# MyrtleSoftware/myrtlespeech

Hardware: AMD Instinct MI355X
Metric: audio-sec/s (RTF), DS2 5xBiLSTM-1024 encoder forward + CTC greedy, 80-feature 10 s clips @ batch 32/GPU (higher is better)
Workload: dtype f16x3 (f32 split in fp16 hi+lo, 3 fp16 MFMA passes, f32 acc: LSTM, projections, conv1/2, FC1; FC2/CTC/decode f32)

## Files before the change

include/ms_hotpath.h:

```cpp
#ifndef MS_HOTPATH_H
#define MS_HOTPATH_H

#include <stddef.h>
#include <stdint.h>

#ifdef __cplusplus
extern "C" {
#endif

#define MS_ABI_VERSION 4

enum {
  MS_OK = 0,
  MS_ERR_INVALID = 1,
  MS_ERR_HIP = 2,
  MS_ERR_WORKSPACE = 3,
  MS_ERR_TIMEOUT = 4,
  MS_ERR_UNSUPPORTED = 5
};

enum { MS_CELL_LSTM = 0, MS_CELL_GRU = 1, MS_CELL_RNN_TANH = 2, MS_CELL_HARD_LSTM = 3 };

enum { MS_ACT_NONE = 0, MS_ACT_CLAMP = 1  };

int ms_abi_version(void);
const char* ms_last_error(void);


int ms_mask_time_(float* x, const int32_t* lens, int N, int inner, int T, void* stream);

size_t ms_maskconv_packed_bytes(int Cout, int Cin_g, int KF, int KT, int groups);

int ms_maskconv_pack(const float* w, void* packed, int Cout, int Cin_g, int KF, int KT, int groups, void* stream);

int ms_maskconv_forward(const float* x, const int32_t* lens, const void* packed_w, const float* bias, float* y,
                        int N, int Cin, int Fin, int Tin, int Cout, int Fout, int Tout, int KF, int KT, int SF,
                        int ST, int DF, int DT, int pad_f_l, int pad_t_l, int groups, int act, float act_lo,
                        float act_hi, void* stream);

size_t ms_maskconv_cl_packed_bytes(int Cout, int Cin, int KF, int KT);
int ms_maskconv_cl_pack(const float* w, void* packed, int Cout, int Cin, int KF, int KT, void* stream);
size_t ms_maskconv_cl_workspace_bytes(int N, int Cin, int Fin, int Tin);
int ms_maskconv_cl_forward(const float* x, const int32_t* lens, const void* packed_w, const float* bias, float* y,
                           int N, int Cin, int Fin, int Tin, int Cout, int Fout, int Tout, int KF, int KT, int SF,
                           int ST, int DF, int DT, int pad_f_l, int pad_t_l, int act, float act_lo, float act_hi,
                           void* workspace, size_t workspace_bytes, void* stream);

size_t ms_maskconv_fwin_packed_bytes(int Cout, int KF, int KT);
int ms_maskconv_fwin_pack(const float* w, void* packed, int Cout, int KF, int KT, void* stream);
size_t ms_maskconv_fwin_workspace_bytes(int N, int Tin, int KF, int SF, int Fout);
int ms_maskconv_fwin_forward(const float* x, const int32_t* lens, const void* packed_w, const float* bias, float* y, int N,
                             int Fin, int Tin, int Cout, int Fout, int Tout, int KF, int KT, int SF, int ST, int DT,
                             int pad_f_l, int pad_t_l, int act, float act_lo, float act_hi, void* workspace,
                             size_t workspace_bytes, void* stream);

size_t ms_maskconv1d_gemm_packed_bytes(int Cout, int Cin, int KT);
int ms_maskconv1d_gemm_pack(const float* w, void* packed, int Cout, int Cin, int KT, void* stream);
size_t ms_maskconv1d_gemm_workspace_bytes(int N, int Cin, int Tout, int Cout, int KT);
int ms_maskconv1d_gemm_forward(const float* x, const int32_t* lens, const void* packed, const float* bias, float* y, int N,
                               int Cin, int Tin, int Cout, int Tout, int KT, int ST, int DT, int pad_l, int act,
                               float act_lo, float act_hi, void* workspace, size_t workspace_bytes, void* stream);

int ms_nct_to_tnc(const float* x, float* y, int N, int CF, int T, void* stream);

int ms_clamp(const float* x, float* y, size_t n, float lo, float hi, void* stream);


int ms_linear_forward(const float* x, const float* w, const float* bias, float* y, int M, int K, int N, int act,
                      float act_lo, float act_hi, void* stream);

#define MS_LINEAR_FEW_ROWS 1
size_t ms_linear_splitk_workspace_bytes(int M, int K, int N, int flags);
int ms_linear_splitk_forward(const float* x, const float* w, const float* bias, float* y, int M, int K, int N, int act,
                             float act_lo, float act_hi, int flags, void* workspace, size_t workspace_bytes, void* stream);

size_t ms_linear_split_workspace_bytes(int M, int K, int N);
int ms_linear_split_forward(const float* x, const float* w, const float* bias, float* y, int M, int K, int N, int act,
                            float act_lo, float act_hi, void* workspace, size_t workspace_bytes, void* stream);

size_t ms_linear_split_packed_bytes(int K, int N);
int ms_linear_split_pack(const float* w, void* packed, int K, int N, void* stream);
int ms_linear_split_forward_packed(const float* x, const void* packed_w, const float* bias, float* y, int M, int K, int N, int act,
                                   float act_lo, float act_hi, void* workspace, size_t workspace_bytes, void* stream);


int ms_lookahead_forward(const float* x, const float* w, float* y, int N, int F, int T, int ctx, long xs_n,
                         long xs_f, long xs_t, long ys_n, long ys_f, long ys_t, int act, float act_lo,
                         float act_hi, void* stream);

int ms_lookahead_window_forward(const float* x, const float* w, float* y, int N, int F, int T_in, int T_out, int ctx,
                                long xs_n, long xs_f, long xs_t, long ys_n, long ys_f, long ys_t, int act, float act_lo,
                                float act_hi, void* stream);


int ms_rnn_padded_hidden(int cell, int H, int ndir);
size_t ms_rnn_packed_bytes(int cell, int In, int H, int ndir);
int ms_rnn_pack(int cell, int In, int H, int ndir, const float* const* w_ih_host, const float* const* w_hh_host,
                const float* const* b_ih_host, const float* const* b_hh_host, void* packed, void* stream);

size_t ms_rnn_workspace_bytes(int cell, int T, int N, int In, int H, int ndir);

int ms_rnn_layer_forward(int cell, const void* packed, const float* x, const int32_t* lens, int max_len,
                         const float* h0, const float* c0, float* out, float* hn, float* cn, int T, int N, int In,
                         int H, int ndir, void* workspace, size_t workspace_bytes, void* stream);

enum { MS_RNN_X_PLANES_IN_WS = 1, MS_RNN_OUT_PLANES_TO_WS = 2, MS_RNN_PACKED_ROWS = 4, MS_RNN_HX_PREINIT = 4096,
       MS_RNN_RECURRENCE_ONLY = 8192, MS_RNN_TIMING_SKIP_PROJECTION = 8192 ,
       MS_RNN_PROJECTION_ONLY = 16384 };
int ms_rnn_layer_chains_planes(int cell, int H, int ndir);
int ms_rnn_hx_preinit(int cell, int T, int N, int In, int H, int ndir, int max_len, int nregions, void* workspace,
                      size_t workspace_bytes, void* stream);
int ms_rnn_layer_packs_rows(int cell, int T, int N, int In, int H, int ndir);
int ms_rnn_layer_forward_ex(int cell, const void* packed, const float* x, const int32_t* lens, int max_len,
                            const float* h0, const float* c0, float* out, float* hn, float* cn, int T, int N, int In,
                            int H, int ndir, int flags, void* workspace, size_t workspace_bytes, void* stream);

int ms_rnn_layer_is_wide(int cell, int H, int ndir, int N);
int ms_rnn_stack_overlap_ok(int cell, int T, int N, int In, int H, int ndir, int nl);
int ms_rnn_stack_forward(int cell, const void* const* packed_host, const float* x, const int32_t* lens, int max_len,
                         const float* h0, const float* c0, float* out, float* hn, float* cn, int T, int N, int In, int H, int ndir,
                         int nl, int segments, void* workspace, size_t workspace_bytes, void* stream);

int ms_rnn_status(const void* workspace, void* stream);

size_t ms_rnn_debug_offset(int cell, int T, int N, int In, int H, int ndir);

int ms_gemm_set_variant(int variant);

enum {
  MS_PROF_PROJECTION = 0, MS_PROF_RECURRENCE = 1, MS_PROF_GEMM_K_LARGE = 2, MS_PROF_GEMM_K_SMALL = 3, MS_PROF_CONV = 4,
  MS_PROF_LAYOUT = 5, MS_PROF_LINEAR = 6, MS_PROF_GREEDY = 7, MS_PROF_OTHER = 8
};
#define MS_PROF_KINDS 9
int ms_prof_enable(int on);
int ms_prof_read(float* out_ms_host, int* out_n_host);

int ms_clock_probe(unsigned long long* out_dev, int samples, int spacing_us, void* stream);

int ms_barrier_chain_probe(unsigned long long* out_dev, int steps, int threads, void* stream);


size_t ms_ctc_loss_workspace_bytes(int T, int N, int V, int S_max);

int ms_ctc_status(const void* workspace, void* stream);

#define MS_CTC_LOG_PROBS_IN 2
int ms_ctc_loss_forward(const float* logits, const int32_t* in_lens, const int32_t* targets,
                        const int32_t* tgt_offsets, const int32_t* tgt_lens, float* nll, float* reduced, int T,
                        int N, int V, int S_max, int blank, int reduction, int zero_infinity, void* workspace,
                        size_t workspace_bytes, void* stream);

int ms_log_softmax_axis(const float* x, float* y, int outer, int axis, int inner, void* stream);
int ms_log_softmax_axis_backward(const float* y, const float* g, float* gx, int outer, int axis, int inner, void* stream);

size_t ms_ctc_loss_backward_workspace_bytes(int T, int N, int V, int S_max);
int ms_ctc_loss_backward(const float* logits, const int32_t* in_lens, const int32_t* targets, const int32_t* tgt_offsets,
                         const int32_t* tgt_lens, const float* grad_nll, float* grad_logits, int T, int N, int V,
                         int S_max, int blank, int zero_infinity, void* workspace, size_t workspace_bytes, void* stream);


int ms_ctc_greedy_decode(const float* x, const int32_t* lens, int32_t* out_idx, int32_t* out_len, int T, int N,
                         int V, int blank, void* stream);

size_t ms_ctc_greedy_stream_state_bytes(int N);
int ms_ctc_greedy_stream_begin(void* state, int N, void* stream);
int ms_ctc_greedy_stream_step(const float* x, int rows, int n, int V, int blank, const int32_t* total_lens,
                              const int32_t* chunk_lens, int32_t* labels, int32_t* label_frames, int cap, int32_t* fresh,
                              void* state, int N, void* stream);


#define MS_CTC_ALIGN_BP_LDS_BYTES 98304
size_t ms_ctc_align_workspace_bytes(int T, int N, int V, int S_max);
int ms_ctc_align(const float* x, const int32_t* in_lens, const int32_t* targets, const int32_t* tgt_offsets,
                 const int32_t* tgt_lens, float* score, int32_t* frame_state, int32_t* token_start, int32_t* token_end,
                 float* token_logp, int T, int N, int V, int L_max, int blank, int flags, void* workspace,
                 size_t workspace_bytes, void* stream);


size_t ms_ctc_beam_workspace_bytes(int T, int N, int V, int beam_width);

int ms_ctc_beam_decode(const float* probs, const int32_t* lens, int32_t* out_idx, int32_t* out_len, int T, int N,
                       int V, int blank, int beam_width, float prune_threshold, int separator, const float* word_factor,
                       int t_begin, int t_end, const float* lm_factor, int finish, int32_t* beam_len,
                       int32_t* beam_idx, int32_t* beam_plen, void* workspace, size_t workspace_bytes,
                       void* stream);

int ms_ctc_beam_decode_rows(const float* probs, const int32_t* lens, int32_t* out_idx, int32_t* out_len, int T, int N,
                            int V, int blank, int beam_width, float prune_threshold, int separator,
                            const float* word_factor, int t_begin, int t_end, int row0, int rows_held,
                            const float* lm_factor, int finish, int32_t* beam_len, int32_t* beam_idx, int32_t* beam_plen,
                            void* workspace, size_t workspace_bytes, void* stream);


#define MS_NGRAM_MAX_ORDER 5

int ms_ngram_lm_table_check(const void* blob_host, size_t bytes);

int ms_ngram_lm_score(const void* table, const void* header_host, size_t table_bytes, const int32_t* prefixes,
                      const int32_t* prefix_lens, float* out, int P, int L, int separator, void* stream);

size_t ms_ctc_beam_lm_workspace_bytes(int T, int N, int V, int beam_width, int order);
int ms_ctc_beam_decode_lm(const float* probs, const int32_t* lens, int32_t* out_idx, int32_t* out_len, int T, int N,
                          int V, int blank, int beam_width, float prune_threshold, int separator,
                          const float* word_factor, int t_begin, int t_end, int row0, int rows_held, const void* lm_table,
                          const void* lm_header_host, size_t lm_table_bytes, int finish, int32_t* beam_len,
                          int32_t* beam_idx, int32_t* beam_plen, void* workspace, size_t workspace_bytes, void* stream);

int ms_ctc_beam_decode_ex(const float* probs, const int32_t* lens, int32_t* out_idx, int32_t* out_len, int T, int N,
                          int V, int blank, int beam_width, float prune_threshold, int separator,
                          const float* word_factor, int t_begin, int t_end, int row0, int rows_held,
                          const float* lm_factor, int finish, int32_t* beam_len, int32_t* beam_idx, int32_t* beam_plen,
                          void* workspace, size_t workspace_bytes, void* stream, const void* lm_table,
                          const void* lm_header_host, size_t lm_table_bytes, int range_safe, float* beam_score,
                          int32_t* scale_log2);


size_t ms_mfcc_workspace_bytes(int N, int T, int n_fft, int n_mels, int n_mfcc);
int ms_mfcc_forward(const float* wave, const int32_t* wave_lens, const float* window, const float* dft,
                    const float* mel_fb, const float* dct, float* out, int N, int max_samples, int T, int n_fft,
                    int hop, int n_mels, int n_mfcc, float top_db, void* workspace, size_t workspace_bytes,
                    void* stream);

int ms_mfcc_legacy_forward(const float* wave, const int32_t* wave_lens, const double* twiddle, const double* fbank,
                           const double* dct, const double* lifter, float* out, int N, int max_samples, int T,
                           int frame_len, int frame_step, int nfft, int nfilt, int numcep, double preemph,
                           void* stream);

size_t ms_standardize_workspace_bytes(int N);
int ms_standardize_forward(const float* x, const int32_t* lens, float* y, int N, int inner, int T, void* workspace,
                           size_t workspace_bytes, void* stream);

int ms_context_frames_forward(const float* x, const int32_t* lens, float* y, int N, int F, int T, int n_context,
                              void* stream);

int ms_spec_augment_(float* x, const int32_t* f_bands, const int32_t* t_bands, int N, int C, int F, int T, int n_f,
                     int n_t, void* stream);


int ms_embedding_forward(const float* table, const int32_t* idx, float* out, int R, int D, int V1, void* stream);

int ms_rnnt_joint_forward(const float* enc_p, const int32_t* enc_row, const float* pred_p, const float* w_out,
                          const float* b_out, float* logp, int R, int J, int V1, void* stream);

int ms_rnnt_topk(const float* scores, int32_t* out_idx, float* out_val, int B, int C, int k, void* stream);

size_t ms_rnnt_decode_workspace_bytes(int T, int N, int V, int D, int H, int L, int J, int beam_width, int max_symbols,
                                      int greedy);
int ms_rnnt_decode(const float* enc_p, const int32_t* lens, const float* embedding, const float* const* w_ih,
                   const float* const* w_hh, const float* const* b_ih, const float* const* b_hh, const float* w_pred,
                   const float* w_out, const float* b_out, int32_t* out_idx, int32_t* out_len, float* out_score, int T,
                   int N, int V, int D, int H, int L, int J, int beam_width, int max_symbols, int greedy, void* workspace,
                   size_t workspace_bytes, void* stream);

size_t ms_rnnt_loss_lattice_bytes(int N, int T, int U1);
size_t ms_rnnt_loss_workspace_bytes(int N, int T, int U1, int V1);
int ms_rnnt_loss_forward(const float* logits, const int32_t* in_lens, const int32_t* targets, const int32_t* tgt_lens,
                         float* nll, float* lattice, int N, int T, int U1, int V1, int blank, void* workspace,
                         size_t workspace_bytes, void* stream);
int ms_rnnt_loss_backward(const float* logits, const int32_t* in_lens, const int32_t* targets, const int32_t* tgt_lens,
                          const float* nll, const float* lattice, const float* grad_nll, float* grad, int N, int T, int U1,
                          int V1, int blank, void* stream);

size_t ms_rnnt_score_lattice_bytes(int N, int T, int U1);
size_t ms_rnnt_score_workspace_bytes(int N, int T, int U1, int J, int V1);
int ms_rnnt_score(const float* enc_p, const float* pred_p, const float* w_out, const float* b_out, const int32_t* in_lens,
                  const int32_t* targets, const int32_t* tgt_lens, float* nll, float* lattice, int N, int T, int U1, int J,
                  int V1, int blank, void* workspace, size_t workspace_bytes, void* stream);

#ifdef __cplusplus
}
#endif
#endif
```

myrtlespeech_amd/_lib.py:

```python
import ctypes
import os
import re
from ctypes import POINTER, c_char_p, c_double, c_float, c_int, c_int32, c_long, c_size_t, c_void_p

import torch

_HERE = os.path.dirname(os.path.abspath(__file__))
LIB_PATH = os.environ.get("MS_HOTPATH_LIB") or os.path.join(_HERE, "libms_hotpath.so")
HEADER_PATH = os.path.join(os.path.dirname(_HERE), "include", "ms_hotpath.h")

MS_OK = 0
ABI_VERSION = 4
ERR_NAMES = {1: "MS_ERR_INVALID", 2: "MS_ERR_HIP", 3: "MS_ERR_WORKSPACE", 4: "MS_ERR_TIMEOUT", 5: "MS_ERR_UNSUPPORTED"}

CELL_LSTM, CELL_GRU, CELL_RNN_TANH, CELL_HARD_LSTM = 0, 1, 2, 3
ACT_NONE, ACT_CLAMP = 0, 1
LINEAR_FEW_ROWS = 1
PROF_KINDS = 9

_P = c_void_p
_PP = POINTER(c_void_p)

SIGNATURES = {
    "ms_abi_version": (c_int, []),
    "ms_last_error": (c_char_p, []),
    "ms_mask_time_": (c_int, [_P, _P, c_int, c_int, c_int, _P]),
    "ms_maskconv_packed_bytes": (c_size_t, [c_int, c_int, c_int, c_int, c_int]),
    "ms_maskconv_pack": (c_int, [_P, _P, c_int, c_int, c_int, c_int, c_int, _P]),
    "ms_maskconv_forward": (c_int, [_P, _P, _P, _P, _P] + [c_int] * 17 + [c_float, c_float, _P]),
    "ms_maskconv_cl_packed_bytes": (c_size_t, [c_int, c_int, c_int, c_int]),
    "ms_maskconv_cl_pack": (c_int, [_P, _P, c_int, c_int, c_int, c_int, _P]),
    "ms_maskconv_cl_workspace_bytes": (c_size_t, [c_int, c_int, c_int, c_int]),
    "ms_maskconv_cl_forward": (c_int, [_P, _P, _P, _P, _P] + [c_int] * 16 + [c_float, c_float, _P, c_size_t, _P]),
    "ms_maskconv_fwin_packed_bytes": (c_size_t, [c_int, c_int, c_int]),
    "ms_maskconv_fwin_pack": (c_int, [_P, _P, c_int, c_int, c_int, _P]),
    "ms_maskconv_fwin_workspace_bytes": (c_size_t, [c_int, c_int, c_int, c_int, c_int]),
    "ms_maskconv_fwin_forward": (c_int, [_P, _P, _P, _P, _P] + [c_int] * 14 + [c_float, c_float, _P, c_size_t, _P]),
    "ms_maskconv1d_gemm_packed_bytes": (c_size_t, [c_int, c_int, c_int]),
    "ms_maskconv1d_gemm_pack": (c_int, [_P, _P, c_int, c_int, c_int, _P]),
    "ms_maskconv1d_gemm_workspace_bytes": (c_size_t, [c_int] * 5),
    "ms_maskconv1d_gemm_forward": (c_int, [_P, _P, _P, _P, _P] + [c_int] * 10 + [c_float, c_float, _P, c_size_t, _P]),
    "ms_nct_to_tnc": (c_int, [_P, _P, c_int, c_int, c_int, _P]),
    "ms_clamp": (c_int, [_P, _P, c_size_t, c_float, c_float, _P]),
    "ms_linear_forward": (c_int, [_P, _P, _P, _P, c_int, c_int, c_int, c_int, c_float, c_float, _P]),
    "ms_linear_splitk_workspace_bytes": (c_size_t, [c_int, c_int, c_int, c_int]),
    "ms_linear_splitk_forward": (c_int, [_P, _P, _P, _P, c_int, c_int, c_int, c_int, c_float, c_float, c_int, _P, c_size_t, _P]),
    "ms_linear_split_workspace_bytes": (c_size_t, [c_int, c_int, c_int]),
    "ms_linear_split_forward": (c_int, [_P, _P, _P, _P, c_int, c_int, c_int, c_int, c_float, c_float, _P, c_size_t, _P]),
    "ms_linear_split_packed_bytes": (c_size_t, [c_int, c_int]),
    "ms_linear_split_pack": (c_int, [_P, _P, c_int, c_int, _P]),
    "ms_linear_split_forward_packed": (c_int, [_P, _P, _P, _P, c_int, c_int, c_int, c_int, c_float, c_float, _P, c_size_t, _P]),
    "ms_lookahead_forward": (c_int, [_P, _P, _P, c_int, c_int, c_int, c_int] + [c_long] * 6 + [c_int, c_float, c_float, _P]),
    "ms_lookahead_window_forward": (c_int, [_P, _P, _P, c_int, c_int, c_int, c_int, c_int] + [c_long] * 6 + [c_int, c_float, c_float, _P]),
    "ms_rnn_packed_bytes": (c_size_t, [c_int, c_int, c_int, c_int]),
    "ms_ctc_status": (c_int, [_P, _P]),
    "ms_rnn_padded_hidden": (c_int, [c_int, c_int, c_int]),
    "ms_rnn_hx_preinit": (c_int, [c_int] * 8 + [_P, c_size_t, _P]),
    "ms_rnn_pack": (c_int, [c_int, c_int, c_int, c_int, _PP, _PP, _PP, _PP, _P, _P]),
    "ms_rnn_workspace_bytes": (c_size_t, [c_int] * 6),
    "ms_rnn_layer_forward": (c_int, [c_int, _P, _P, _P, c_int, _P, _P, _P, _P, _P] + [c_int] * 5 + [_P, c_size_t, _P]),
    "ms_rnn_layer_forward_ex": (c_int, [c_int, _P, _P, _P, c_int, _P, _P, _P, _P, _P] + [c_int] * 6 + [_P, c_size_t, _P]),
    "ms_rnn_layer_chains_planes": (c_int, [c_int, c_int, c_int]),
    "ms_rnn_layer_is_wide": (c_int, [c_int] * 4),
    "ms_rnn_stack_overlap_ok": (c_int, [c_int] * 7),
    "ms_rnn_stack_forward": (c_int, [c_int, _P, _P, _P, c_int, _P, _P, _P, _P, _P] + [c_int] * 7 + [_P, c_size_t, _P]),
    "ms_rnn_status": (c_int, [_P, _P]),
    "ms_rnn_debug_offset": (c_size_t, [c_int] * 6),
    "ms_rnn_layer_packs_rows": (c_int, [c_int] * 6),
    "ms_gemm_set_variant": (c_int, [c_int]),
    "ms_prof_enable": (c_int, [c_int]),
    "ms_prof_read": (c_int, [POINTER(c_float), POINTER(c_int)]),
    "ms_clock_probe": (c_int, [_P, c_int, c_int, _P]),
    "ms_barrier_chain_probe": (c_int, [_P, c_int, c_int, _P]),
    "ms_ctc_loss_workspace_bytes": (c_size_t, [c_int] * 4),
    "ms_ctc_loss_forward": (c_int, [_P] * 7 + [c_int] * 7 + [_P, c_size_t, _P]),
    "ms_log_softmax_axis": (c_int, [_P, _P, c_int, c_int, c_int, _P]),
    "ms_log_softmax_axis_backward": (c_int, [_P, _P, _P, c_int, c_int, c_int, _P]),
    "ms_ctc_loss_backward_workspace_bytes": (c_size_t, [c_int] * 4),
    "ms_ctc_loss_backward": (c_int, [_P] * 7 + [c_int] * 6 + [_P, c_size_t, _P]),
    "ms_ctc_greedy_decode": (c_int, [_P, _P, _P, _P, c_int, c_int, c_int, c_int, _P]),
    "ms_ctc_align_workspace_bytes": (c_size_t, [c_int] * 4),
    "ms_ctc_align": (c_int, [_P] * 10 + [c_int] * 6 + [_P, c_size_t, _P]),
    "ms_ctc_greedy_stream_state_bytes": (c_size_t, [c_int]),
    "ms_ctc_greedy_stream_begin": (c_int, [_P, c_int, _P]),
    "ms_ctc_greedy_stream_step": (c_int, [_P, c_int, c_int, c_int, c_int, _P, _P, _P, _P, c_int, _P, _P, c_int, _P]),
    "ms_embedding_forward": (c_int, [_P, _P, _P, c_int, c_int, c_int, _P]),
    "ms_rnnt_joint_forward": (c_int, [_P, _P, _P, _P, _P, _P, c_int, c_int, c_int, _P]),
    "ms_rnnt_topk": (c_int, [_P, _P, _P, c_int, c_int, c_int, _P]),
    "ms_ctc_beam_workspace_bytes": (c_size_t, [c_int] * 4),
    "ms_ctc_beam_decode": (c_int, [_P, _P, _P, _P, c_int, c_int, c_int, c_int, c_int, c_float, c_int, _P, c_int, c_int,
                                   _P, c_int, _P, _P, _P, _P, c_size_t, _P]),
    "ms_ctc_beam_decode_rows": (c_int, [_P, _P, _P, _P, c_int, c_int, c_int, c_int, c_int, c_float, c_int, _P, c_int, c_int,
                                        c_int, c_int, _P, c_int, _P, _P, _P, _P, c_size_t, _P]),
    "ms_ngram_lm_table_check": (c_int, [_P, c_size_t]),
    "ms_ngram_lm_score": (c_int, [_P, _P, c_size_t, _P, _P, _P, c_int, c_int, c_int, _P]),
    "ms_ctc_beam_lm_workspace_bytes": (c_size_t, [c_int] * 5),
    "ms_ctc_beam_decode_lm": (c_int, [_P, _P, _P, _P, c_int, c_int, c_int, c_int, c_int, c_float, c_int, _P, c_int, c_int,
                                      c_int, c_int, _P, _P, c_size_t, c_int, _P, _P, _P, _P, c_size_t, _P]),
    "ms_ctc_beam_decode_ex": (c_int, [_P, _P, _P, _P, c_int, c_int, c_int, c_int, c_int, c_float, c_int, _P, c_int, c_int,
                                      c_int, c_int, _P, c_int, _P, _P, _P, _P, c_size_t, _P, _P, _P, c_size_t, c_int, _P, _P]),
    "ms_rnnt_decode_workspace_bytes": (c_size_t, [c_int] * 10),
    "ms_rnnt_decode": (c_int, [_P, _P, _P, _PP, _PP, _PP, _PP, _P, _P, _P, _P, _P, _P] + [c_int] * 10 + [_P, c_size_t, _P]),
    "ms_rnnt_loss_lattice_bytes": (c_size_t, [c_int] * 3),
    "ms_rnnt_loss_workspace_bytes": (c_size_t, [c_int] * 4),
    "ms_rnnt_loss_forward": (c_int, [_P] * 6 + [c_int] * 5 + [_P, c_size_t, _P]),
    "ms_rnnt_loss_backward": (c_int, [_P] * 8 + [c_int] * 5 + [_P]),
    "ms_rnnt_score_lattice_bytes": (c_size_t, [c_int] * 3),
    "ms_rnnt_score_workspace_bytes": (c_size_t, [c_int] * 5),
    "ms_rnnt_score": (c_int, [_P] * 9 + [c_int] * 6 + [_P, c_size_t, _P]),
    "ms_mfcc_workspace_bytes": (c_size_t, [c_int] * 5),
    "ms_mfcc_forward": (c_int, [_P] * 7 + [c_int] * 7 + [c_float, _P, c_size_t, _P]),
    "ms_mfcc_legacy_forward": (c_int, [_P] * 7 + [c_int] * 8 + [c_double, _P]),
    "ms_standardize_workspace_bytes": (c_size_t, [c_int]),
    "ms_standardize_forward": (c_int, [_P, _P, _P, c_int, c_int, c_int, _P, c_size_t, _P]),
    "ms_context_frames_forward": (c_int, [_P, _P, _P, c_int, c_int, c_int, c_int, _P]),
    "ms_spec_augment_": (c_int, [_P, _P, _P] + [c_int] * 6 + [_P]),
}

_lib = None


def header_symbols():
    with open(HEADER_PATH) as f:
        text = re.sub(r"/\*.*?\*/", "", f.read(), flags=re.S)
    return sorted(set(re.findall(r"\b(ms_[a-z0-9_]+)\s*\(", text)))


def load():
    global _lib
    if _lib is None:
        if not os.path.exists(LIB_PATH):
            raise RuntimeError(
                f"{LIB_PATH} not found: build it with `python -c 'import __graft_entry__ as g; g.build()'` "
                "(or `make -C myrtlespeech_amd/csrc`). There is no CPU fallback."
            )
        lib = ctypes.CDLL(LIB_PATH)
        for name, (res, args) in SIGNATURES.items():
            fn = getattr(lib, name)
            fn.restype = res
            fn.argtypes = args
        got = lib.ms_abi_version()
        if got != ABI_VERSION:
            raise RuntimeError(f"{LIB_PATH} reports MS_ABI_VERSION {got}, this binding needs {ABI_VERSION}: rebuild the "
                               "library (`make -C myrtlespeech_amd/csrc`)")
        _lib = lib
    return _lib


def require_gpu():
    if not torch.cuda.is_available():
        raise RuntimeError("myrtlespeech_amd: a HIP device (MI355X) is required; there is no CPU fallback")


def stream_ptr():
    return c_void_p(torch.cuda.current_stream().cuda_stream)


def ptr(t, strided=False):
    if t is None:
        return c_void_p(0)
    if not isinstance(t, torch.Tensor):
        raise TypeError(f"_lib.ptr: expected a torch.Tensor or None, got {type(t).__name__}")
    if not t.is_cuda:
        raise ValueError(f"_lib.ptr: a {t.device.type} tensor (shape {tuple(t.shape)}) cannot be a device-pointer argument; "
                         "move it to the GPU first (host buffers go through _lib.host_ptr)")
    if not strided and not t.is_contiguous():
        raise ValueError(f"_lib.ptr: tensor of shape {tuple(t.shape)} and strides {tuple(t.stride())} is not contiguous; the "
                         "kernels read dense storage (call .contiguous())")
    return c_void_p(t.data_ptr())


def host_ptr(t):
    if t is None:
        return c_void_p(0)
    if not isinstance(t, torch.Tensor) or t.is_cuda or not t.is_contiguous():
        raise ValueError("_lib.host_ptr: expected a contiguous CPU tensor")
    return c_void_p(t.data_ptr())


def check(rc, what):
    if rc != MS_OK:
        msg = load().ms_last_error().decode()
        raise RuntimeError(f"{what} failed with {ERR_NAMES.get(rc, rc)}: {msg}")


def f32c(t):
    if t.dtype != torch.float32:
        t = t.float()
    if not t.is_cuda:
        t = t.cuda()
    return t.contiguous()


_ASYNC_LENS = os.environ.get("MS_ASYNC_LENS") != "0"


_const_lens = {}


def _const_tensor(shape, dtype, value, make: bool):
    key = (tuple(shape), dtype, int(value))
    rec = _const_lens.get(key)
    if rec is not None:
        t, version = rec
        if version_of(t) == version:
            return t
        _const_lens[("stale", len(_const_lens)) + key] = rec
        del _const_lens[key]
    if not make or len(_const_lens) >= 4096:
        return None
    t = torch.full(tuple(shape), int(value), dtype=dtype, device="cuda")
    _const_lens[key] = (t, version_of(t))
    return t


def _all_equal_value(h: torch.Tensor):
    if h.numel() == 0 or h.numel() > 4096 or h.dtype not in (torch.int32, torch.int64):
        return None
    flat = h.reshape(-1)
    v = int(flat[0])
    return v if bool((flat == v).all()) else None


def upload(host: torch.Tensor, dtype=None) -> torch.Tensor:
    h = host.detach()
    if dtype is not None and h.dtype != dtype:
        h = h.to(dtype)
    h = h.contiguous()
    if torch.cuda.is_available() and torch.cuda.is_current_stream_capturing():
        flat = h.reshape(-1)
        if flat.numel() and bool((flat == flat[0]).all()):
            c = _const_tensor(h.shape, h.dtype, flat[0].item(), make=False) if h.dtype in (torch.int32, torch.int64) else None
            return c if c is not None else torch.full(h.shape, flat[0].item(), dtype=h.dtype, device="cuda")
        raise RuntimeError("host values that differ cannot be uploaded inside a HIP graph capture")
    if torch.cuda.is_available():
        v = _all_equal_value(h)
        if v is not None:
            _const_tensor(h.shape, h.dtype, v, make=True)
    if not _ASYNC_LENS:
        return h.cuda()
    try:
        h = h.pin_memory()
    except RuntimeError:
        return h.cuda()
    return h.to("cuda", non_blocking=True)


def attach_host(dev: torch.Tensor, host: torch.Tensor) -> torch.Tensor:
    dev._ms_host = (host.detach().clone(), version_of(dev), dev.data_ptr())
    return dev


def version_of(t: torch.Tensor) -> int:
    return -1 if t.is_inference() else t._version


def host_lens(lens: torch.Tensor) -> torch.Tensor:
    if not lens.is_cuda:
        return lens.detach().to(torch.int64)
    h = cached_host(lens) if _ASYNC_LENS else None
    if h is not None:
        return h.to(torch.int64)
    return lens.detach().to("cpu", torch.int64)


def cached_host(lens: torch.Tensor):
    rec = getattr(lens, "_ms_host", None)
    if rec is None:
        return None
    h, version, address = rec
    if h.shape == lens.shape and version == version_of(lens) and address == lens.data_ptr():
        return h
    lens._ms_host = None
    return None


def lens_to_device(lens: torch.Tensor) -> torch.Tensor:
    if lens.is_cuda:
        return lens
    return attach_host(upload(lens), lens.detach())


def lens_i32(lens):
    if lens.is_cuda:
        if lens.dtype == torch.int32 and lens.is_contiguous():
            return lens
        h = cached_host(lens) if _ASYNC_LENS else None
        if h is not None:
            v = _all_equal_value(h)
            if v is not None:
                c = _const_tensor(lens.shape, torch.int32, v, make=not torch.cuda.is_current_stream_capturing())
                if c is not None and torch.cuda.is_current_stream_capturing():
                    return c
        return lens.to(torch.int32).contiguous()
    return upload(lens, torch.int32)


def split_precision():
    return os.environ.get("MS_PRECISION") != "f32"


issue_point = None


def at_issue_point():
    hook = issue_point
    if hook is not None:
        hook()


class Workspace:

    def __init__(self):
        self.buf = None

    def get(self, nbytes, zero: bool = True):
        if self.buf is None or self.buf.numel() < nbytes:
            make = torch.zeros if zero else torch.empty
            self.buf = make(max(int(nbytes), 256), dtype=torch.uint8, device="cuda")
        return self.buf
```

myrtlespeech_amd/csrc/conv_cl.hip:

```cpp
#include <algorithm>
#include <type_traits>

#include "common.h"

namespace {

typedef unsigned u32x4 __attribute__((ext_vector_type(4)));
typedef unsigned u32x2 __attribute__((ext_vector_type(2)));
typedef __bf16 bf16x8 __attribute__((ext_vector_type(8)));
typedef _Float16 f16x8 __attribute__((ext_vector_type(8)));

constexpr int CL_F = 2;

struct ClP {
  int N, Cin, Fin, Tin, Cout, Fout, Tout, KF, KT, SF, ST, DF, DT, pad_f, pad_t;
  int KG;
  int PW;
  int co_tiles;
  int act;
  float lo, hi;
  int FP;
};

__device__ __forceinline__ unsigned bf16b(float x) { return (unsigned)__builtin_bit_cast(unsigned short, (__bf16)x); }
__device__ __forceinline__ unsigned f16b(float x) { return (unsigned)__builtin_bit_cast(unsigned short, (_Float16)x); }
__device__ __forceinline__ void split_by_prec(float x, int prec, unsigned& hi, unsigned& lo) {
  if (prec == ms::PREC_F16) { hi = f16b(x); lo = 0u; }
  else if (prec == ms::PREC_F16X3) ms::plane_split<true>(x, hi, lo);
  else ms::plane_split<false>(x, hi, lo);
}

__global__ void conv_cl_pack_kernel(const float* __restrict__ w, unsigned short* __restrict__ packed, int Cout, int Cin,
                                    int KF, int KT, int cout_pad, int prec, const float* __restrict__ scale_word) {
  const int KG = Cin / 8;
  const float wscale = scale_word[0];
  const size_t plane = (size_t)KF * KT * KG * cout_pad * 8;
  for (size_t i = (size_t)blockIdx.x * blockDim.x + threadIdx.x; i < plane; i += (size_t)gridDim.x * blockDim.x) {
    const int e = i & 7;
    const int co = (i >> 3) % cout_pad;
    const int kg = (i / ((size_t)8 * cout_pad)) % KG;
    const int kt = (i / ((size_t)8 * cout_pad * KG)) % KT;
    const int kf = i / ((size_t)8 * cout_pad * KG * KT);
    float x = 0.f;
    if (co < Cout) x = w[(((size_t)co * Cin + kg * 8 + e) * KF + kf) * KT + kt] * wscale;
    unsigned h, l;
    split_by_prec(x, prec, h, l);
    packed[i] = (unsigned short)h;
    packed[plane + i] = (unsigned short)l;
  }
}

template <int P, bool WIN = false, int WF = 1>
__global__ __launch_bounds__(256, 2) void maskconv_cl_kernel(const unsigned short* __restrict__ xh,
                                                             const unsigned short* __restrict__ xl,
                                                             const int32_t* __restrict__ lens,
                                                             const unsigned short* __restrict__ wp,
                                                             const float* __restrict__ bias, float* __restrict__ y, ClP p,
                                                             const float* __restrict__ scale_word) {
  constexpr bool F16 = ms::prec_one_plane(P), HM = P == ms::PREC_F16X3;
  constexpr int WT = 4 / WF;
  constexpr int TT = 32 * WT;
  constexpr int RF = CL_F * WF;
  extern __shared__ __attribute__((aligned(16))) char lds[];
  const int row_bytes = p.KG * p.PW * 16;
  char* Ph = lds;
  char* Pl = lds + RF * row_bytes;
  char* Wh = lds + 2 * RF * row_bytes;
  const int wtap = p.KG * 32 * 16;
  char* Wl = Wh + ((p.KT + 1) / 2) * wtap;

  const int tid = threadIdx.x, lane = tid & 63, wave = tid >> 6;
  const int l31 = lane & 31, half = lane >> 5;
  const int wt = wave % WT, wf = wave / WT;
  const int t0 = blockIdx.x * TT;
  const int fo0 = blockIdx.y * RF;
  const int n = blockIdx.z / p.co_tiles, tile = blockIdx.z % p.co_tiles;
  const int len = lens ? min(lens[n], p.Tin) : p.Tin;
  const int cout_pad = p.co_tiles * 32;
  const size_t wplane = (size_t)p.KF * p.KT * p.KG * cout_pad * 8;

  ms::f32x16 acc[CL_F];
#pragma unroll
  for (int f = 0; f < CL_F; ++f)
#pragma unroll
    for (int r = 0; r < 16; ++r) acc[f][r] = 0.f;

  const int tin0 = t0 * p.ST - p.pad_t;
  const int ngran = p.KG * p.PW;
  const unsigned plane_bytes = WIN ? (unsigned)((size_t)p.N * p.Tin * p.FP * 2) : 0u;
  const __amdgpu_buffer_rsrc_t xh_rsrc = __builtin_amdgcn_make_buffer_rsrc(const_cast<unsigned short*>(xh), 0, plane_bytes, 0x00020000);
  const __amdgpu_buffer_rsrc_t xl_rsrc = __builtin_amdgcn_make_buffer_rsrc(const_cast<unsigned short*>(xl), 0, plane_bytes, 0x00020000);

  for (int kf = 0; kf < p.KF; ++kf) {
    for (int f = 0; f < RF; ++f) {
      const int fin = (fo0 + f) * p.SF - p.pad_f + kf * p.DF;
      const bool frow = (fo0 + f) < p.Fout && (WIN || (fin >= 0 && fin < p.Fin));
      const size_t rbase = ((size_t)n * p.Fin + (frow && !WIN ? fin : 0)) * p.Tin;
      for (int i = tid; i < ngran; i += 256) {
        const int q = i / p.KG, kg = i - q * p.KG;
        const int tin = tin0 + q;
        u32x4 vh = {0u, 0u, 0u, 0u}, vl = {0u, 0u, 0u, 0u};
        if (frow && tin >= 0 && tin < len) {
          if (WIN) {
            const int boff = (int)((((size_t)n * p.Tin + tin) * p.FP + (size_t)(fo0 + f) * p.SF + kg * 8) * 2);
            vh = __builtin_amdgcn_raw_buffer_load_b128(xh_rsrc, boff, 0, 0);
            if (!F16) vl = __builtin_amdgcn_raw_buffer_load_b128(xl_rsrc, boff, 0, 0);
          } else {
            const size_t off = (rbase + tin) * p.Cin + kg * 8;
            vh = *reinterpret_cast<const u32x4*>(xh + off);
            if (!F16) vl = *reinterpret_cast<const u32x4*>(xl + off);
          }
        }
        *reinterpret_cast<u32x4*>(Ph + f * row_bytes + (kg * p.PW + q) * 16) = vh;
        if (!F16) *reinterpret_cast<u32x4*>(Pl + f * row_bytes + (kg * p.PW + q) * 16) = vl;
      }
    }
    const int taps_per_stage = (p.KT + 1) / 2;
    for (int kt0 = 0; kt0 < p.KT; kt0 += taps_per_stage) {
      const int ntap = min(taps_per_stage, p.KT - kt0);
      if (kt0 > 0) __syncthreads();
      {
        const int ng = ntap * p.KG * 32;
        for (int i = tid; i < ng; i += 256) {
          const int co = i & 31, rest = i >> 5;
          const size_t src = ((((size_t)kf * p.KT + kt0) * p.KG + rest) * cout_pad + tile * 32 + co) * 8;
          *reinterpret_cast<u32x4*>(Wh + i * 16) = *reinterpret_cast<const u32x4*>(wp + src);
          if (!F16) *reinterpret_cast<u32x4*>(Wl + i * 16) = *reinterpret_cast<const u32x4*>(wp + wplane + src);
        }
      }
      __syncthreads();
      for (int ktl = 0; ktl < ntap; ++ktl) {
        const int tq = (wt * 32 + l31) * p.ST + (kt0 + ktl) * p.DT;
        for (int s = 0; s < p.KG / 2; ++s) {
          const int kg = 2 * s + half;
          const int woff = ((ktl * p.KG + kg) * 32 + l31) * 16;
          const u32x4 ah = *reinterpret_cast<const u32x4*>(Wh + woff);
          u32x4 al = ah;
          if (!F16) al = *reinterpret_cast<const u32x4*>(Wl + woff);
#pragma unroll
          for (int f = 0; f < CL_F; ++f) {
            const int poff = (wf * CL_F + f) * row_bytes + (kg * p.PW + tq) * 16;
            const u32x4 bh = *reinterpret_cast<const u32x4*>(Ph + poff);
            if (F16) {
              acc[f] = __builtin_amdgcn_mfma_f32_32x32x16_f16(__builtin_bit_cast(f16x8, ah), __builtin_bit_cast(f16x8, bh), acc[f], 0, 0, 0);
            } else {
              const u32x4 bl = *reinterpret_cast<const u32x4*>(Pl + poff);
              acc[f] = ms::mfma_32x32x16<HM>(ah, bh, acc[f]);
              acc[f] = ms::mfma_32x32x16<HM>(al, bh, acc[f]);
              acc[f] = ms::mfma_32x32x16<HM>(ah, bl, acc[f]);
            }
          }
        }
      }
    }
    __syncthreads();
  }

  const int t = t0 + wt * 32 + l31;
  const float winv = scale_word[1];
  if (t < p.Tout) {
#pragma unroll
    for (int f = 0; f < CL_F; ++f) {
      const int fo = fo0 + wf * CL_F + f;
      if (fo >= p.Fout) continue;
#pragma unroll
      for (int r = 0; r < 16; ++r) {
        const int co = tile * 32 + ms::mfma32_row(r, lane);
        if (co < p.Cout) {
          float v = acc[f][r] * winv + (bias ? bias[co] : 0.f);
          if (p.act == MS_ACT_CLAMP) v = fminf(fmaxf(v, p.lo), p.hi);
          y[(((size_t)n * p.Cout + co) * p.Fout + fo) * p.Tout + t] = v;
        }
      }
    }
  }
}


constexpr int SH_RB = 12;
constexpr int SH_KT = 11;

template <int P>
__global__ __launch_bounds__(256, 1) void maskconv_cl_short_kernel(const unsigned short* __restrict__ xh,
                                                                   const unsigned short* __restrict__ xl,
                                                                   const int32_t* __restrict__ lens,
                                                                   const unsigned short* __restrict__ wp,
                                                                   const float* __restrict__ bias, float* __restrict__ y, ClP p,
                                                                   int RB, int RIN, const float* __restrict__ scale_word) {
  constexpr bool F16 = ms::prec_one_plane(P), HM = P == ms::PREC_F16X3;
  const float winv = scale_word[1];
  extern __shared__ __attribute__((aligned(16))) char lds[];
  const int tid = threadIdx.x, lane = tid & 63, wave = __builtin_amdgcn_readfirstlane(tid >> 6);
  const int c16 = lane & 15, q = lane >> 4;
  const int fo0 = blockIdx.x * RB, cb = blockIdx.y, n = blockIdx.z;
  const int PW = p.PW;
  const int row_bytes = PW * 64;
  char* Ph = lds;
  char* Pl = lds + (size_t)RIN * row_bytes;
  const int len = lens ? min(lens[n], p.Tin) : p.Tin;
  const int fin_lo = fo0 * p.SF - p.pad_f;

  for (int i = tid; i < RIN * PW * 4; i += 256) {
    const int kg = i & 3, rq = i >> 2;
    const int r = rq / PW, fq = rq - r * PW;
    const int fin = fin_lo + r, tin = fq - p.pad_t;
    u32x4 vh = {0u, 0u, 0u, 0u}, vl = {0u, 0u, 0u, 0u};
    if (fin >= 0 && fin < p.Fin && tin >= 0 && tin < len) {
      const size_t off = (((size_t)n * p.Fin + fin) * p.Tin + tin) * 32 + kg * 8;
      vh = *reinterpret_cast<const u32x4*>(xh + off);
      if (!F16) vl = *reinterpret_cast<const u32x4*>(xl + off);
    }
    *reinterpret_cast<u32x4*>(Ph + r * row_bytes + fq * 64 + kg * 16) = vh;
    if (!F16) *reinterpret_cast<u32x4*>(Pl + r * row_bytes + fq * 64 + kg * 16) = vl;
  }
  __syncthreads();

  ms::f32x4 acc[SH_RB];
#pragma unroll
  for (int i = 0; i < SH_RB; ++i) acc[i] = ms::f32x4{0.f, 0.f, 0.f, 0.f};
  const int cout_pad = p.co_tiles * 32;
  const size_t wplane = (size_t)p.KF * p.KT * 4 * cout_pad * 8;
  const unsigned short* wa = wp + (size_t)q * cout_pad * 8 + (cb * 16 + c16) * 8;
  const size_t tap_stride = (size_t)4 * cout_pad * 8;
  u32x4 fh[2][SH_KT], fl[2][SH_KT];
  auto load_row = [&](auto set, int kf) {
#pragma unroll
    for (int kt = 0; kt < SH_KT; ++kt)
      if (kt < p.KT) {
        const unsigned short* src = wa + (size_t)(kf * p.KT + kt) * tap_stride;
        fh[set][kt] = *reinterpret_cast<const u32x4*>(src);
        if (!F16) fl[set][kt] = *reinterpret_cast<const u32x4*>(src + wplane);
      }
  };
  auto compute_row = [&](auto set, int kf) {
#pragma unroll
    for (int i = 0; i < SH_RB; ++i) {
      const int fo = fo0 + i;
      const int fin = fo * p.SF - p.pad_f + kf * p.DF;
      if (i < RB && fo < p.Fout && fin >= 0 && fin < p.Fin) {
        const int rbase = (fin - fin_lo) * row_bytes + c16 * 64 + q * 16;
#pragma unroll
        for (int kt = 0; kt < SH_KT; ++kt)
          if (kt < p.KT) {
            const u32x4 bh = *reinterpret_cast<const u32x4*>(Ph + rbase + kt * 64);
            if (F16) {
              acc[i] = __builtin_amdgcn_mfma_f32_16x16x32_f16(__builtin_bit_cast(f16x8, fh[set][kt]), __builtin_bit_cast(f16x8, bh), acc[i], 0, 0, 0);
            } else {
              const u32x4 bl = *reinterpret_cast<const u32x4*>(Pl + rbase + kt * 64);
              acc[i] = ms::mfma_16x16x32<HM>(fh[set][kt], bh, acc[i]);
              acc[i] = ms::mfma_16x16x32<HM>(fl[set][kt], bh, acc[i]);
              acc[i] = ms::mfma_16x16x32<HM>(fh[set][kt], bl, acc[i]);
            }
          }
      }
    }
  };
  constexpr std::integral_constant<int, 0> S0{};
  constexpr std::integral_constant<int, 1> S1{};
  if (wave < p.KF) load_row(S0, wave);
  for (int kf = wave; kf < p.KF; kf += 8) {
    if (kf + 4 < p.KF) load_row(S1, kf + 4);
    compute_row(S0, kf);
    if (kf + 8 < p.KF) load_row(S0, kf + 8);
    if (kf + 4 < p.KF) compute_row(S1, kf + 4);
  }

  __syncthreads();
  ms::f32x4* part = reinterpret_cast<ms::f32x4*>(lds);
#pragma unroll
  for (int i = 0; i < SH_RB; ++i)
    if (i < RB) part[(wave * SH_RB + i) * 64 + lane] = acc[i];
  __syncthreads();
#pragma unroll
  for (int j = 0; j < SH_RB / 4; ++j) {
    const int i = wave + 4 * j, fo = fo0 + i;
    if (i >= RB || fo >= p.Fout) continue;
    ms::f32x4 v = part[(0 * SH_RB + i) * 64 + lane];
#pragma unroll
    for (int w = 1; w < 4; ++w) v += part[(w * SH_RB + i) * 64 + lane];
    if (c16 < p.Tout) {
#pragma unroll
      for (int r = 0; r < 4; ++r) {
        const int co = cb * 16 + 4 * q + r;
        if (co < p.Cout) {
          float o = v[r] * winv + (bias ? bias[co] : 0.f);
          if (p.act == MS_ACT_CLAMP) o = fminf(fmaxf(o, p.lo), p.hi);
          y[(((size_t)n * p.Cout + co) * p.Fout + fo) * p.Tout + c16] = o;
        }
      }
    }
  }
}

int conv_cl_short_plan(const ClP& p, bool f16, int* RB, int* RIN, size_t* lds) {
  static const bool off = getenv("MS_CONV_SHORT") && getenv("MS_CONV_SHORT")[0] == '0';
  if (off || p.Cin != 32 || p.Tout > 16 || p.ST != 1 || p.DT != 1 || p.FP != 0 || p.N > 65535 || p.KT > SH_KT) return 0;
  const int cbs = ms::cdiv(p.Cout, 16);
  int nblk = std::max(1, std::min(ms::cdiv(p.Fout, 4), ms::cdiv(ms::num_cus(), p.N * cbs)));
  while (ms::cdiv(p.Fout, nblk) > SH_RB) ++nblk;
  for (; nblk <= p.Fout; ++nblk) {
    const int rb = ms::cdiv(p.Fout, nblk);
    const int rin = (rb - 1) * p.SF + (p.KF - 1) * p.DF + 1;
    const size_t bytes = std::max((size_t)(f16 ? 1 : 2) * rin * (p.Tout + p.KT - 1) * 64, (size_t)4 * SH_RB * 64 * 16);
    if (bytes <= 156 * 1024) { *RB = rb; *RIN = rin; *lds = bytes; return 1; }
  }
  return 0;
}

__global__ void nchw_to_cl_split_kernel(const float* __restrict__ x, unsigned short* __restrict__ hi,
                                        unsigned short* __restrict__ lo, int C, int F, int T, int prec) {
  __shared__ float tile[32][33];
  const int n = blockIdx.z / F, f = blockIdx.z % F;
  const int t0 = blockIdx.x * 32, c0 = blockIdx.y * 32;
  const int tx = threadIdx.x, ty = threadIdx.y;
  for (int i = ty; i < 32; i += 8) {
    const int c = c0 + i, t = t0 + tx;
    tile[i][tx] = (c < C && t < T) ? x[(((size_t)n * C + c) * F + f) * T + t] : 0.f;
  }
  __syncthreads();
  for (int i = ty; i < 32; i += 8) {
    const int t = t0 + i, c = c0 + tx;
    if (t < T && c < C) {
      const float v = tile[tx][i];
      const size_t o = (((size_t)n * F + f) * T + t) * C + c;
      unsigned h, l;
      split_by_prec(v, prec, h, l);
      hi[o] = (unsigned short)h;
      if (prec != ms::PREC_F16) lo[o] = (unsigned short)l;
    }
  }
}

__global__ void ft_to_tf_split_kernel(const float* __restrict__ x, unsigned short* __restrict__ hi,
                                      unsigned short* __restrict__ lo, int Fin, int T, int FP, int pad, int prec) {
  __shared__ float tile[32][33];
  const int n = blockIdx.z;
  const int t0 = blockIdx.x * 32, j0 = blockIdx.y * 32;
  const int tx = threadIdx.x, ty = threadIdx.y;
  for (int i = ty; i < 32; i += 8) {
    const int fidx = j0 + i - pad, t = t0 + tx;
    tile[i][tx] = (fidx >= 0 && fidx < Fin && t < T) ? x[((size_t)n * Fin + fidx) * T + t] : 0.f;
  }
  __syncthreads();
  for (int i = ty; i < 32; i += 8) {
    const int t = t0 + i, j = j0 + tx;
    if (t < T && j < FP) {
      const float v = tile[tx][i];
      const size_t o = ((size_t)n * T + t) * FP + j;
      unsigned h, l;
      split_by_prec(v, prec, h, l);
      hi[o] = (unsigned short)h;
      if (prec != ms::PREC_F16) lo[o] = (unsigned short)l;
    }
  }
}

__global__ void conv_fwin_pack_kernel(const float* __restrict__ w, unsigned short* __restrict__ packed, int Cout, int KF,
                                      int KT, int KG, int cout_pad, int prec, const float* __restrict__ scale_word) {
  const size_t plane = (size_t)KT * KG * cout_pad * 8;
  const float wscale = scale_word[0];
  for (size_t i = (size_t)blockIdx.x * blockDim.x + threadIdx.x; i < plane; i += (size_t)gridDim.x * blockDim.x) {
    const int e = i & 7;
    const int co = (i >> 3) % cout_pad;
    const int kg = (i / ((size_t)8 * cout_pad)) % KG;
    const int kt = i / ((size_t)8 * cout_pad * KG);
    const int kf = kg * 8 + e;
    float x = 0.f;
    if (co < Cout && kf < KF) x = w[((size_t)co * KF + kf) * KT + kt] * wscale;
    unsigned h, l;
    split_by_prec(x, prec, h, l);
    packed[i] = (unsigned short)h;
    packed[plane + i] = (unsigned short)l;
  }
}

int conv_cl_plan(ClP& p, size_t* lds) {
  const size_t wbytes = (size_t)2 * ((p.KT + 1) / 2) * p.KG * 32 * 16;
  if ((long)p.N * p.co_tiles > 65535) return 0;
  for (int wf : {p.Tout <= 48 ? 4 : 1, 1}) {
    const int tt = 128 / wf, rf = CL_F * wf;
    p.PW = (tt - 1) * p.ST + (p.KT - 1) * p.DT + 1;
    *lds = (size_t)2 * rf * p.KG * p.PW * 16 + wbytes;
    if (*lds <= 160 * 1024 && ms::cdiv(p.Fout, rf) <= 65535) return wf;
  }
  return 0;
}

template <bool WIN>
int conv_cl_launch(const ClP& p, int wf, size_t lds, const unsigned short* xh, const unsigned short* xl, const int32_t* lens,
                   const void* packed_w, const float* bias, float* y, hipStream_t stream, const float* scale_word) {
  static ms::DeviceOnce attr_once;
  if (attr_once.need()) {
#define MS_CL_ATTR(PP)                                                                                                                     \
    MS_HIP(hipFuncSetAttribute((const void*)maskconv_cl_kernel<PP, WIN, 1>, hipFuncAttributeMaxDynamicSharedMemorySize, 160 * 1024));   \
    MS_HIP(hipFuncSetAttribute((const void*)maskconv_cl_kernel<PP, WIN, 4>, hipFuncAttributeMaxDynamicSharedMemorySize, 160 * 1024));
    MS_CL_ATTR(ms::PREC_BF16X3) MS_CL_ATTR(ms::PREC_F16) MS_CL_ATTR(ms::PREC_F16X3)
#undef MS_CL_ATTR
    attr_once.done();
  }
  const int prec = ms::split_mode();
  const int tt = 128 / wf, rf = CL_F * wf;
  dim3 grid(ms::cdiv(p.Tout, tt), ms::cdiv(p.Fout, rf), p.N * p.co_tiles);
  const unsigned short* wq = (const unsigned short*)packed_w;
#define MS_CL_LAUNCH(WF_)                                                                                                             \
  if (prec == ms::PREC_F16) hipLaunchKernelGGL((maskconv_cl_kernel<ms::PREC_F16, WIN, WF_>), grid, dim3(256), lds, stream, xh, xl, lens, wq, bias, y, p, scale_word); \
  else if (prec == ms::PREC_F16X3) hipLaunchKernelGGL((maskconv_cl_kernel<ms::PREC_F16X3, WIN, WF_>), grid, dim3(256), lds, stream, xh, xl, lens, wq, bias, y, p, scale_word); \
  else hipLaunchKernelGGL((maskconv_cl_kernel<ms::PREC_BF16X3, WIN, WF_>), grid, dim3(256), lds, stream, xh, xl, lens, wq, bias, y, p, scale_word);
  if (wf == 4) { MS_CL_LAUNCH(4) } else { MS_CL_LAUNCH(1) }
#undef MS_CL_LAUNCH
  MS_LAUNCH_CHECK();
  return MS_OK;
}

inline int fwin_kfp(int KF) { return ms::cdiv(KF, 16) * 16; }
inline int fwin_fp(int KF, int SF, int Fout) { return ms::cdiv((Fout - 1) * SF + fwin_kfp(KF), 32) * 32; }

}

static size_t fwin_plane_bytes(int Cout, int KF, int KT) {
  return ms::align_up((size_t)2 * KT * (fwin_kfp(KF) / 8) * (ms::cdiv(Cout, 32) * 32) * 8 * sizeof(unsigned short), 256);
}
extern "C" size_t ms_maskconv_fwin_packed_bytes(int Cout, int KF, int KT) {
  if (Cout <= 0 || KF <= 0 || KT <= 0) return 0;
  return fwin_plane_bytes(Cout, KF, KT) + 256;
}

extern "C" int ms_maskconv_fwin_pack(const float* w, void* packed, int Cout, int KF, int KT, void* stream) {
  MS_REQUIRE(w && packed, "null pointer");
  MS_REQUIRE(Cout > 0 && KF > 0 && KT > 0, "bad shape");
  const int cout_pad = ms::cdiv(Cout, 32) * 32, KG = fwin_kfp(KF) / 8;
  const size_t plane = (size_t)KT * KG * cout_pad * 8;
  const int blocks = (int)std::min<size_t>((plane + 255) / 256, 2048);
  float* scale_word = (float*)((char*)packed + fwin_plane_bytes(Cout, KF, KT));
  const int rc = ms::weight_scale_launch(w, (size_t)Cout * KF * KT, scale_word, ms::split_mode(), (hipStream_t)stream);
  if (rc != MS_OK) return rc;
  hipLaunchKernelGGL(conv_fwin_pack_kernel, dim3(blocks), dim3(256), 0, (hipStream_t)stream, w, (unsigned short*)packed, Cout,
                     KF, KT, KG, cout_pad, ms::split_mode(), scale_word);
  MS_LAUNCH_CHECK();
  return MS_OK;
}

extern "C" size_t ms_maskconv_fwin_workspace_bytes(int N, int Tin, int KF, int SF, int Fout) {
  if (N <= 0 || Tin <= 0 || KF <= 0 || SF <= 0 || Fout <= 0) return 0;
  return ms::align_up((size_t)N * Tin * fwin_fp(KF, SF, Fout) * 4, 256);
}

extern "C" int ms_maskconv_fwin_forward(const float* x, const int32_t* lens, const void* packed_w, const float* bias, float* y,
                                        int N, int Fin, int Tin, int Cout, int Fout, int Tout, int KF, int KT, int SF, int ST,
                                        int DT, int pad_f_l, int pad_t_l, int act, float act_lo, float act_hi, void* workspace,
                                        size_t workspace_bytes, void* stream_) {
  ms::ProfScope prof_span(MS_PROF_CONV, (hipStream_t)stream_);
  MS_REQUIRE(x && packed_w && y && workspace, "null pointer");
  MS_REQUIRE(N > 0 && Fin > 0 && Tin > 0 && Cout > 0 && Fout > 0 && Tout > 0, "bad shape");
  MS_REQUIRE(KF > 0 && KT > 0 && SF > 0 && ST > 0 && DT > 0 && pad_f_l >= 0 && pad_t_l >= 0, "bad kernel");
  MS_REQUIRE(SF % 2 == 0, "feature stride must be even (4-byte aligned window loads)");
  MS_REQUIRE(act == MS_ACT_NONE || act == MS_ACT_CLAMP, "bad act");
  if (workspace_bytes < ms_maskconv_fwin_workspace_bytes(N, Tin, KF, SF, Fout)) {
    ms::set_error("ms_maskconv_fwin_forward: workspace too small");
    return MS_ERR_WORKSPACE;
  }
  hipStream_t stream = (hipStream_t)stream_;
  ClP p;
  p.N = N; p.Cin = fwin_kfp(KF); p.Fin = 1; p.Tin = Tin; p.Cout = Cout; p.Fout = Fout; p.Tout = Tout; p.KF = 1; p.KT = KT;
  p.SF = SF; p.ST = ST; p.DF = 1; p.DT = DT; p.pad_f = 0; p.pad_t = pad_t_l; p.KG = p.Cin / 8;
  p.co_tiles = ms::cdiv(Cout, 32);
  p.act = act; p.lo = act_lo; p.hi = act_hi;
  p.FP = fwin_fp(KF, SF, Fout);
  size_t lds = 0;
  const int wf = conv_cl_plan(p, &lds);
  if (wf == 0 || (size_t)N * Tin * p.FP * 2 >= ((size_t)1 << 31)) {
    ms::set_error("ms_maskconv_fwin_forward: shape outside the LDS / grid budget");
    return MS_ERR_UNSUPPORTED;
  }
  unsigned short* xh = (unsigned short*)workspace;
  unsigned short* xl = xh + (size_t)N * Tin * p.FP;
  const int prec = ms::split_mode();
  const bool f16 = prec == ms::PREC_F16;
  hipLaunchKernelGGL(ft_to_tf_split_kernel, dim3(ms::cdiv(Tin, 32), ms::cdiv(p.FP, 32), N), dim3(32, 8), 0, stream, x, xh, xl,
                     Fin, Tin, p.FP, pad_f_l, prec);
  MS_LAUNCH_CHECK();
  return conv_cl_launch<true>(p, wf, lds, xh, xl, lens, packed_w, bias, y, stream,
                              (const float*)((const char*)packed_w + fwin_plane_bytes(Cout, KF, KT)));
}

static size_t cl_plane_bytes(int Cout, int Cin, int KF, int KT) {
  return ms::align_up((size_t)2 * KF * KT * (Cin / 8) * (ms::cdiv(Cout, 32) * 32) * 8 * sizeof(unsigned short), 256);
}
extern "C" size_t ms_maskconv_cl_packed_bytes(int Cout, int Cin, int KF, int KT) {
  if (Cout <= 0 || Cin <= 0 || Cin % 16 || KF <= 0 || KT <= 0) return 0;
  return cl_plane_bytes(Cout, Cin, KF, KT) + 256;
}

extern "C" int ms_maskconv_cl_pack(const float* w, void* packed, int Cout, int Cin, int KF, int KT, void* stream) {
  MS_REQUIRE(w && packed, "null pointer");
  MS_REQUIRE(Cout > 0 && Cin > 0 && Cin % 16 == 0 && KF > 0 && KT > 0, "bad shape (Cin must be a multiple of 16)");
  const int cout_pad = ms::cdiv(Cout, 32) * 32;
  const size_t plane = (size_t)KF * KT * (Cin / 8) * cout_pad * 8;
  const int blocks = (int)std::min<size_t>((plane + 255) / 256, 2048);
  float* scale_word = (float*)((char*)packed + cl_plane_bytes(Cout, Cin, KF, KT));
  const int rc = ms::weight_scale_launch(w, (size_t)Cout * Cin * KF * KT, scale_word, ms::split_mode(), (hipStream_t)stream);
  if (rc != MS_OK) return rc;
  hipLaunchKernelGGL(conv_cl_pack_kernel, dim3(blocks), dim3(256), 0, (hipStream_t)stream, w, (unsigned short*)packed, Cout,
                     Cin, KF, KT, cout_pad, ms::split_mode(), scale_word);
  MS_LAUNCH_CHECK();
  return MS_OK;
}

extern "C" size_t ms_maskconv_cl_workspace_bytes(int N, int Cin, int Fin, int Tin) {
  if (N <= 0 || Cin <= 0 || Fin <= 0 || Tin <= 0) return 0;
  return ms::align_up((size_t)N * Cin * Fin * Tin * 4, 256);
}

extern "C" int ms_maskconv_cl_forward(const float* x, const int32_t* lens, const void* packed_w, const float* bias, float* y,
                                      int N, int Cin, int Fin, int Tin, int Cout, int Fout, int Tout, int KF, int KT,
                                      int SF, int ST, int DF, int DT, int pad_f_l, int pad_t_l, int act, float act_lo,
                                      float act_hi, void* workspace, size_t workspace_bytes, void* stream_) {
  ms::ProfScope prof_span(MS_PROF_CONV, (hipStream_t)stream_);
  MS_REQUIRE(x && packed_w && y && workspace, "null pointer");
  MS_REQUIRE(N > 0 && Cin > 0 && Cin % 16 == 0 && Fin > 0 && Tin > 0 && Cout > 0 && Fout > 0 && Tout > 0, "bad shape");
  MS_REQUIRE(KF > 0 && KT > 0 && SF > 0 && ST > 0 && DF > 0 && DT > 0 && pad_f_l >= 0 && pad_t_l >= 0, "bad kernel");
  MS_REQUIRE(act == MS_ACT_NONE || act == MS_ACT_CLAMP, "bad act");
  if (workspace_bytes < ms_maskconv_cl_workspace_bytes(N, Cin, Fin, Tin)) {
    ms::set_error("ms_maskconv_cl_forward: workspace too small");
    return MS_ERR_WORKSPACE;
  }
  hipStream_t stream = (hipStream_t)stream_;
  ClP p;
  p.N = N; p.Cin = Cin; p.Fin = Fin; p.Tin = Tin; p.Cout = Cout; p.Fout = Fout; p.Tout = Tout; p.KF = KF; p.KT = KT;
  p.SF = SF; p.ST = ST; p.DF = DF; p.DT = DT; p.pad_f = pad_f_l; p.pad_t = pad_t_l; p.KG = Cin / 8;
  p.co_tiles = ms::cdiv(Cout, 32);
  p.act = act; p.lo = act_lo; p.hi = act_hi;
  p.FP = 0;
  size_t lds = 0;
  const int wf = conv_cl_plan(p, &lds);
  if (wf == 0) {
    ms::set_error("ms_maskconv_cl_forward: shape outside the LDS / grid budget");
    return MS_ERR_UNSUPPORTED;
  }
  const float* scale_word = (const float*)((const char*)packed_w + cl_plane_bytes(Cout, Cin, KF, KT));
  unsigned short* xh = (unsigned short*)workspace;
  unsigned short* xl = xh + (size_t)N * Cin * Fin * Tin;
  MS_REQUIRE(N * Fin <= 65535, "N*Fin exceeds grid limits");
  const int prec = ms::split_mode();
  const bool f16 = prec == ms::PREC_F16;
  hipLaunchKernelGGL(nchw_to_cl_split_kernel, dim3(ms::cdiv(Tin, 32), ms::cdiv(Cin, 32), N * Fin), dim3(32, 8), 0, stream, x,
                     xh, xl, Cin, Fin, Tin, prec);
  MS_LAUNCH_CHECK();
  {
    int RB = 0, RIN = 0;
    size_t slds = 0;
    if (conv_cl_short_plan(p, f16, &RB, &RIN, &slds)) {
      static ms::DeviceOnce attr_once;
      if (attr_once.need()) {
        MS_HIP(hipFuncSetAttribute((const void*)maskconv_cl_short_kernel<ms::PREC_BF16X3>, hipFuncAttributeMaxDynamicSharedMemorySize, 160 * 1024));
        MS_HIP(hipFuncSetAttribute((const void*)maskconv_cl_short_kernel<ms::PREC_F16>, hipFuncAttributeMaxDynamicSharedMemorySize, 160 * 1024));
        MS_HIP(hipFuncSetAttribute((const void*)maskconv_cl_short_kernel<ms::PREC_F16X3>, hipFuncAttributeMaxDynamicSharedMemorySize, 160 * 1024));
        attr_once.done();
      }
      ClP ps = p;
      ps.PW = Tout + KT - 1;
      const dim3 grid(ms::cdiv(Fout, RB), ms::cdiv(Cout, 16), N);
      const unsigned short* wq = (const unsigned short*)packed_w;
      auto kern = prec == ms::PREC_F16 ? maskconv_cl_short_kernel<ms::PREC_F16>
                  : prec == ms::PREC_F16X3 ? maskconv_cl_short_kernel<ms::PREC_F16X3> : maskconv_cl_short_kernel<ms::PREC_BF16X3>;
      hipLaunchKernelGGL(kern, grid, dim3(256), slds, stream, xh, xl, lens, wq, bias, y, ps, RB, RIN, scale_word);
      MS_LAUNCH_CHECK();
      return MS_OK;
    }
  }
  return conv_cl_launch<false>(p, wf, lds, xh, xl, lens, packed_w, bias, y, stream, scale_word);
}
```

myrtlespeech_amd/model/cnn.py:

```python
from enum import Enum
import os
from typing import List, Optional, Tuple, TypeVar, Union

import torch

from myrtlespeech_amd import _lib


class PaddingMode(Enum):

    NONE = 0
    SAME = 1


def pad_same(length: int, kernel_size: int, stride: int = 1, dilation: int = 1) -> Tuple[int, int]:
    for name, v in (("length", length), ("kernel_size", kernel_size), ("stride", stride), ("dilation", dilation)):
        if v <= 0:
            raise ValueError(f"{name}={v} must be > 0")
    span = dilation * (kernel_size - 1) + 1
    n_out = (length + stride - 1) // stride
    total = stride * n_out - 1 + span - length
    left = total // 2
    return left, total - left


def out_lens(seq_lens: torch.Tensor, kernel_size: int, stride: int, dilation: int, padding: int) -> torch.Tensor:
    v = seq_lens.to(torch.float32)
    v = (v + float(padding) - float(dilation * (kernel_size - 1) + 1)) / float(stride) + 1.0
    return v.floor().to(seq_lens.dtype)


def _pair(v):
    return (int(v[0]), int(v[1])) if isinstance(v, (list, tuple)) else (int(v), int(v))


class _PackedFilters:

    def __init__(self):
        self.key = None
        self.buf = None
        self.key_cl = None
        self.buf_cl = None
        self.workspace = _lib.Workspace()

    def get_cl(self, weight: torch.Tensor) -> torch.Tensor:
        key = (weight.data_ptr(), _lib.version_of(weight), tuple(weight.shape))
        if key != self.key_cl:
            lib = _lib.load()
            cout, cin, kf, kt = weight.shape
            self.buf_cl = torch.empty(lib.ms_maskconv_cl_packed_bytes(cout, cin, kf, kt), dtype=torch.uint8, device="cuda")
            w = _lib.f32c(weight.detach())
            _lib.check(lib.ms_maskconv_cl_pack(_lib.ptr(w), _lib.ptr(self.buf_cl), cout, cin, kf, kt, _lib.stream_ptr()),
                       "ms_maskconv_cl_pack")
            self.key_cl = key
        return self.buf_cl

    def get_fwin(self, weight: torch.Tensor) -> torch.Tensor:
        key = (weight.data_ptr(), _lib.version_of(weight), tuple(weight.shape), "fwin")
        if key != self.key_cl:
            lib = _lib.load()
            cout, _, kf, kt = weight.shape
            self.buf_cl = torch.empty(lib.ms_maskconv_fwin_packed_bytes(cout, kf, kt), dtype=torch.uint8, device="cuda")
            w = _lib.f32c(weight.detach())
            _lib.check(lib.ms_maskconv_fwin_pack(_lib.ptr(w), _lib.ptr(self.buf_cl), cout, kf, kt, _lib.stream_ptr()),
                       "ms_maskconv_fwin_pack")
            self.key_cl = key
        return self.buf_cl

    def get_gemm1d(self, weight: torch.Tensor) -> torch.Tensor:
        key = (weight.data_ptr(), _lib.version_of(weight), tuple(weight.shape), "gemm1d")
        if key != self.key_cl:
            lib = _lib.load()
            cout, cin, _, kt = weight.shape
            self.buf_cl = torch.empty(lib.ms_maskconv1d_gemm_packed_bytes(cout, cin, kt), dtype=torch.uint8, device="cuda")
            w = _lib.f32c(weight.detach())
            _lib.check(lib.ms_maskconv1d_gemm_pack(_lib.ptr(w), _lib.ptr(self.buf_cl), cout, cin, kt, _lib.stream_ptr()),
                       "ms_maskconv1d_gemm_pack")
            self.key_cl = key
        return self.buf_cl

    def get(self, weight: torch.Tensor, groups: int) -> torch.Tensor:
        key = (weight.data_ptr(), _lib.version_of(weight), tuple(weight.shape), groups)
        if key != self.key:
            lib = _lib.load()
            cout, cin_g, kf, kt = weight.shape
            nbytes = lib.ms_maskconv_packed_bytes(cout, cin_g, kf, kt, groups)
            self.buf = torch.empty(nbytes, dtype=torch.uint8, device="cuda")
            w = _lib.f32c(weight.detach())
            _lib.check(lib.ms_maskconv_pack(_lib.ptr(w), _lib.ptr(self.buf), cout, cin_g, kf, kt, groups,
                                            _lib.stream_ptr()), "ms_maskconv_pack")
            self.key = key
        return self.buf


def _conv_forward(x4: torch.Tensor, seq_lens: torch.Tensor, weight4: torch.Tensor, bias: Optional[torch.Tensor],
                  packed: _PackedFilters, stride, dilation, groups: int, same: bool,
                  act: Optional[Tuple[float, float]], time_pads: Optional[Tuple[int, int]] = None):
    lib = _lib.load()
    n, cin, fin, tin = x4.shape
    cout, _, kf, kt = weight4.shape
    (sf, st), (df, dt) = stride, dilation
    if same:
        pt = pad_same(tin, kt, st, dt)
        pf = pad_same(fin, kf, sf, df)
    else:
        pt = pf = (0, 0)
    if time_pads is not None:
        pt = (int(time_pads[0]), int(time_pads[1]))
    fout = (fin + sum(pf) - (df * (kf - 1) + 1)) // sf + 1
    tout = (tin + sum(pt) - (dt * (kt - 1) + 1)) // st + 1
    if fout <= 0 or tout <= 0:
        raise RuntimeError("convolution output would be empty")
    host_in = _lib.host_lens(seq_lens).to(seq_lens.dtype)
    new_host = out_lens(host_in, kt, st, dt, sum(pt))
    new_lens = _lib.attach_host(_lib.upload(new_host), new_host)
    y = torch.empty((n, cout, fout, tout), dtype=torch.float32, device="cuda")
    lens_dev = _lib.lens_i32(seq_lens)
    a, lo, hi = (_lib.ACT_NONE, 0.0, 0.0) if act is None else (_lib.ACT_CLAMP, act[0], act[1])
    b = None if bias is None else _lib.f32c(bias.detach())
    big = 2.0 * y.numel() * cin * kf * kt >= float(os.environ.get("MS_CONV_MFMA_MIN_FLOPS", "1e9"))
    if _lib.split_precision() and groups == 1 and fin == 1 and kf == 1 and sf == 1 and pf == (0, 0) and cin * kt >= 64 and big:
        pk = packed.get_gemm1d(weight4)
        nbytes = lib.ms_maskconv1d_gemm_workspace_bytes(n, cin, tout, cout, kt)
        ws = packed.workspace.get(nbytes)
        _lib.check(lib.ms_maskconv1d_gemm_forward(_lib.ptr(x4), _lib.ptr(lens_dev), _lib.ptr(pk), _lib.ptr(b), _lib.ptr(y), n,
                                                  cin, tin, cout, tout, kt, st, dt, pt[0], a, lo, hi, _lib.ptr(ws), nbytes,
                                                  _lib.stream_ptr()), "ms_maskconv1d_gemm_forward")
        return y, new_lens
    if _lib.split_precision() and groups == 1 and cin % 16 == 0 and big:
        pk = packed.get_cl(weight4)
        ws = packed.workspace.get(lib.ms_maskconv_cl_workspace_bytes(n, cin, fin, tin))
        rc = lib.ms_maskconv_cl_forward(_lib.ptr(x4), _lib.ptr(lens_dev), _lib.ptr(pk), _lib.ptr(b), _lib.ptr(y), n, cin,
                                        fin, tin, cout, fout, tout, kf, kt, sf, st, df, dt, pf[0], pt[0], a, lo, hi,
                                        _lib.ptr(ws), ws.numel(), _lib.stream_ptr())
        if rc != 5:
            _lib.check(rc, "ms_maskconv_cl_forward")
            return y, new_lens
    big_fwin = 2.0 * y.numel() * cin * kf * kt >= float(os.environ.get("MS_CONV_MFMA_MIN_FLOPS", "2e8"))
    if (_lib.split_precision() and groups == 1 and cin == 1 and df == 1 and sf % 2 == 0 and kf >= 16 and big_fwin
            and os.environ.get("MS_CONV_FWIN") != "0"):
        pk = packed.get_fwin(weight4)
        nbytes = lib.ms_maskconv_fwin_workspace_bytes(n, tin, kf, sf, fout)
        ws = packed.workspace.get(nbytes)
        rc = lib.ms_maskconv_fwin_forward(_lib.ptr(x4), _lib.ptr(lens_dev), _lib.ptr(pk), _lib.ptr(b), _lib.ptr(y), n, fin,
                                          tin, cout, fout, tout, kf, kt, sf, st, dt, pf[0], pt[0], a, lo, hi, _lib.ptr(ws),
                                          nbytes, _lib.stream_ptr())
        if rc != 5:
            _lib.check(rc, "ms_maskconv_fwin_forward")
            return y, new_lens
    pk = packed.get(weight4, groups)
    _lib.check(lib.ms_maskconv_forward(_lib.ptr(x4), _lib.ptr(lens_dev), _lib.ptr(pk), _lib.ptr(b), _lib.ptr(y), n, cin,
                                       fin, tin, cout, fout, tout, kf, kt, sf, st, df, dt, pf[0], pt[0], groups, a, lo,
                                       hi, _lib.stream_ptr()), "ms_maskconv_forward")
    return y, new_lens


def _mask_in_place(acts: torch.Tensor, seq_lens: torch.Tensor):
    if acts.is_cuda and acts.dtype == torch.float32 and acts.is_contiguous():
        n, t = acts.shape[0], acts.shape[-1]
        h = _lib.host_lens(seq_lens)
        if h.numel() == n and n and int(h.min()) >= t:
            return True
        inner = acts.numel() // (n * t)
        lens_dev = _lib.lens_i32(seq_lens)
        _lib.check(_lib.load().ms_mask_time_(_lib.ptr(acts), _lib.ptr(lens_dev), n, inner, t, _lib.stream_ptr()),
                   "ms_mask_time_")
        return True
    return False


class MaskConv1d(torch.nn.Conv1d):

    def __init__(self, in_channels: int, out_channels: int, kernel_size: int, stride: int = 1,
                 padding_mode: PaddingMode = PaddingMode.NONE, dilation: int = 1, groups: int = 1, bias: bool = True):
        super().__init__(in_channels=in_channels, out_channels=out_channels, kernel_size=kernel_size, stride=stride,
                         dilation=dilation, groups=groups, bias=bias)
        if padding_mode not in (PaddingMode.NONE, PaddingMode.SAME):
            raise ValueError(f"unknown padding mode {padding_mode}")
        self._padding_mode = padding_mode
        self._packed = _PackedFilters()
        self.use_cuda = torch.cuda.is_available()
        if self.use_cuda:
            super().cuda()

    def forward(self, x: Tuple[torch.Tensor, torch.Tensor],
                fused_activation: Optional[Tuple[float, float]] = None) -> Tuple[torch.Tensor, torch.Tensor]:
        _lib.require_gpu()
        acts, seq_lens = x
        _mask_in_place(acts, seq_lens)
        x4 = _lib.f32c(acts).unsqueeze(2)
        y, new_lens = _conv_forward(x4, seq_lens, self.weight.unsqueeze(2), self.bias, self._packed,
                                    (1, self.stride[0]), (1, self.dilation[0]), self.groups,
                                    self._padding_mode == PaddingMode.SAME, fused_activation)
        return y.squeeze(2), new_lens

    def extra_repr(self) -> str:
        return super().extra_repr() + f", padding_mode={self._padding_mode}"


class MaskConv2d(torch.nn.Conv2d):

    def __init__(self, in_channels: int, out_channels: int, kernel_size: Union[int, List[int]],
                 stride: Union[int, List[int]] = 1, padding_mode: PaddingMode = PaddingMode.NONE, dilation: int = 1,
                 groups: int = 1, bias: bool = True):
        super().__init__(in_channels=in_channels, out_channels=out_channels, kernel_size=kernel_size, stride=stride,
                         dilation=dilation, groups=groups, bias=bias)
        if padding_mode not in (PaddingMode.NONE, PaddingMode.SAME):
            raise ValueError(f"unknown padding mode {padding_mode}")
        self._padding_mode = padding_mode
        self._packed = _PackedFilters()
        self.use_cuda = torch.cuda.is_available()
        if self.use_cuda:
            super().cuda()

    def forward(self, x: Tuple[torch.Tensor, torch.Tensor],
                fused_activation: Optional[Tuple[float, float]] = None) -> Tuple[torch.Tensor, torch.Tensor]:
        _lib.require_gpu()
        acts, seq_lens = x
        _mask_in_place(acts, seq_lens)
        x4 = _lib.f32c(acts)
        y, new_lens = _conv_forward(x4, seq_lens, self.weight, self.bias, self._packed, _pair(self.stride),
                                    _pair(self.dilation), self.groups, self._padding_mode == PaddingMode.SAME,
                                    fused_activation)
        return y, new_lens

    def extra_repr(self) -> str:
        return super().extra_repr() + f", padding_mode={self._padding_mode}"


SeqLenT = TypeVar("SeqLenT", torch.Tensor, Tuple[torch.Tensor, torch.Tensor])


class Conv2dTo1d(torch.nn.Module):

    def __init__(self, seq_len_support: bool = True):
        super().__init__()
        self.seq_len_support = seq_len_support

    def forward(self, x: SeqLenT) -> SeqLenT:
        acts, seq_lens = x if self.seq_len_support else (x, None)
        n, c, f, t = acts.size()
        acts = acts.view(n, c * f, t)
        return (acts, seq_lens) if self.seq_len_support else acts

    def extra_repr(self) -> str:
        return f"seq_len_support={self.seq_len_support}"


class Conv1dTo2d(torch.nn.Module):

    def __init__(self, seq_len_support: bool = True):
        super().__init__()
        self.seq_len_support = seq_len_support

    def forward(self, x: SeqLenT) -> SeqLenT:
        acts, seq_lens = x if self.seq_len_support else (x, None)
        acts = acts.unsqueeze(1)
        return (acts, seq_lens) if self.seq_len_support else acts

    def extra_repr(self) -> str:
        return f"seq_len_support={self.seq_len_support}"
```

myrtlespeech_amd/model/deep_speech_2.py:

```python
from typing import Optional, Tuple

import torch

from myrtlespeech_amd import _lib
from myrtlespeech_amd.model.cnn import Conv1dTo2d, Conv2dTo1d, MaskConv1d, MaskConv2d
from myrtlespeech_amd.model.fully_connected import FullyConnected, linear_stack_plan, run_linear_stack
from myrtlespeech_amd.model.lookahead import Lookahead, lookahead_apply
from myrtlespeech_amd.model.rnn import RNNState
from myrtlespeech_amd.model.seq_len_wrapper import SeqLenWrapper
from myrtlespeech_amd.model.utils import activation_clamp


def _is_plain_activation(m) -> bool:
    return (isinstance(m, SeqLenWrapper) and isinstance(m.module, (torch.nn.Hardtanh, torch.nn.ReLU, torch.nn.Identity))
            and isinstance(m.seq_lens_fn, torch.nn.Identity))


class DeepSpeech2(torch.nn.Module):

    def __init__(self, cnn: Optional[torch.nn.Module], rnn: torch.nn.Module, lookahead: Optional[torch.nn.Module],
                 fully_connected: torch.nn.Module):
        super().__init__()
        self.cnn = cnn
        self.rnn = rnn
        self.lookahead = lookahead
        self.fully_connected = fully_connected
        self.use_cuda = torch.cuda.is_available()
        if self.use_cuda:
            self.cuda()

    def _run_cnn(self, h):
        mods = list(self.cnn) if isinstance(self.cnn, torch.nn.Sequential) else [self.cnn]
        i = 0
        while i < len(mods):
            m = mods[i]
            if isinstance(m, (MaskConv1d, MaskConv2d)) and i + 1 < len(mods) and _is_plain_activation(mods[i + 1]):
                h = m(h, fused_activation=activation_clamp(mods[i + 1].module))
                i += 2
            else:
                h = m(h)
                i += 1
        return h

    @staticmethod
    def _conv_to_rnn_size(x: torch.Tensor) -> torch.Tensor:
        n, c, f, t = x.shape
        x = _lib.f32c(x)
        y = torch.empty((t, n, c * f), dtype=torch.float32, device="cuda")
        _lib.check(_lib.load().ms_nct_to_tnc(_lib.ptr(x), _lib.ptr(y), n, c * f, t, _lib.stream_ptr()), "ms_nct_to_tnc")
        return y

    def _run_lookahead_ntf(self, h_tnf: torch.Tensor):
        la = self.lookahead
        mods = list(la) if isinstance(la, torch.nn.Sequential) else [la]
        if not isinstance(mods[0], Lookahead) or len(mods) > 2:
            return None
        clamp = None
        if len(mods) == 2:
            if not _is_plain_activation(mods[1]):
                return None
            clamp = activation_clamp(mods[1].module)
        t, n, f = h_tnf.shape
        return lookahead_apply(h_tnf, mods[0].weight, (f, 1, n * f), n, f, t, out_layout="ntf", clamp=clamp)

    def forward(self, x: Tuple[torch.Tensor, torch.Tensor], hx: Optional[RNNState] = None
                ) -> Tuple[Tuple[torch.Tensor, torch.Tensor], RNNState]:
        return self.back(self.front(x), hx)

    def front(self, x: Tuple[torch.Tensor, torch.Tensor]) -> Tuple[torch.Tensor, torch.Tensor]:
        _lib.require_gpu()
        h = (x[0].cuda() if not x[0].is_cuda else x[0], x[1])
        if self.cnn is not None:
            h = self._run_cnn(h)
        return self._conv_to_rnn_size(h[0]), h[1]

    def back(self, h: Tuple[torch.Tensor, torch.Tensor], hx: Optional[RNNState] = None
             ) -> Tuple[Tuple[torch.Tensor, torch.Tensor], RNNState]:
        return self.output(*self.recurrent(h, hx))

    def recurrent(self, h: Tuple[torch.Tensor, torch.Tensor], hx: Optional[RNNState] = None):
        _lib.at_issue_point()
        h, hid = self.rnn(h, hx=hx)
        _lib.at_issue_point()
        return h[0], h[1], hid

    def output(self, seq: torch.Tensor, lens: torch.Tensor, hid: RNNState
               ) -> Tuple[Tuple[torch.Tensor, torch.Tensor], RNNState]:
        fc = self.fully_connected
        fused_fc = isinstance(fc, FullyConnected)
        if self.lookahead is not None:
            ntf = self._run_lookahead_ntf(seq) if seq.is_contiguous() else None
            if ntf is None:
                la_out, lens = self.lookahead((seq.permute(1, 2, 0), lens))
                ntf = la_out.transpose(1, 2)
            out, lens = fc((ntf, lens))
            return (out.transpose(0, 1), lens), hid
        if fused_fc:
            t, n, f = seq.shape
            y = run_linear_stack(_lib.f32c(seq).reshape(t * n, f), linear_stack_plan(fc.fully_connected, fc.training))
            return (y.reshape(t, n, -1), _lib.lens_to_device(lens)), hid
        out, lens = fc((seq.transpose(0, 1), lens))
        return (out.transpose(0, 1), lens), hid
```

myrtlespeech_amd/pipeline.py:

```python
import copy
import threading
from typing import Callable, List, Optional, Sequence

import torch

from myrtlespeech_amd import _lib

COTENANT_GEMM_VARIANT = 10


class _Baton:

    def __init__(self, n: int):
        self.cv = threading.Condition()
        self.n = n
        self.turn = 0
        self.active = [True] * n

    def _next_active(self, after: int) -> int:
        for d in range(1, self.n + 1):
            k = (after + d) % self.n
            if self.active[k]:
                return k
        return after

    def wait_turn(self, me: int):
        with self.cv:
            while self.turn != me:
                self.cv.wait()

    def pass_on(self, me: int):
        with self.cv:
            self.turn = self._next_active(me)
            self.cv.notify_all()
        self.wait_turn(me)

    def leave(self, me: int):
        with self.cv:
            self.active[me] = False
            if self.turn == me:
                self.turn = self._next_active(me)
            self.cv.notify_all()


def replica(model: torch.nn.Module) -> torch.nn.Module:
    memo = {id(t): t for t in list(model.parameters()) + list(model.buffers())}
    return copy.deepcopy(model, memo)


class BatchesInFlight:

    def __init__(self, model: torch.nn.Module, post: Optional[Callable] = None, pre: Optional[Callable] = None, depth: int = 2):
        _lib.require_gpu()
        if depth < 2 or depth > 4:
            raise ValueError(f"depth={depth} must be in [2, 4]")
        self.depth = depth
        self.models = tuple([model] + [replica(model) for _ in range(depth - 1)])
        self.streams = tuple(torch.cuda.Stream() for _ in range(depth))
        self.post = post
        self.pre = pre
        from myrtlespeech_amd.model.hard_lstm import HardLSTM
        from myrtlespeech_amd.model.rnn import RNN
        self._stacks = [m for mod in self.models for m in mod.modules() if isinstance(m, (RNN, HardLSTM))]
        self._n_caller_stacks = len(self._stacks) // depth

    def __call__(self, batches: Sequence) -> List:
        lib = _lib.load()
        results: List = [None] * len(batches)
        errors: List = []
        baton = _Baton(self.depth)
        slot_of = {}
        device = torch.cuda.current_device()
        caller = torch.cuda.current_stream()
        ready = torch.cuda.Event()
        ready.record(caller)
        inference = torch.is_inference_mode_enabled()

        def hook():
            me = slot_of.get(threading.get_ident())
            if me is not None:
                baton.pass_on(me)

        def worker(me: int):
            slot_of[threading.get_ident()] = me
            try:
                torch.cuda.set_device(device)
                baton.wait_turn(me)
                with torch.cuda.stream(self.streams[me]), torch.no_grad(), torch.inference_mode(inference):
                    self.streams[me].wait_event(ready)
                    for k in range(me, len(batches), self.depth):
                        if self.pre is not None:
                            self.pre(k)
                        out = self.models[me](batches[k])
                        results[k] = out if self.post is None else self.post(out)
                        baton.pass_on(me)
            except BaseException as e:
                errors.append(e)
            finally:
                baton.leave(me)

        prev_hook = _lib.issue_point
        _lib.issue_point = hook
        lib.ms_gemm_set_variant(self._gemm_variant(lib, batches))
        prev_check = [m.check_status for m in self._stacks]
        for m in self._stacks:
            m.check_status = False
        try:
            threads = [threading.Thread(target=worker, args=(m,), daemon=True) for m in range(self.depth)]
            for t in threads:
                t.start()
            for t in threads:
                t.join()
        finally:
            for m, c in zip(self._stacks, prev_check):
                m.check_status = c
            lib.ms_gemm_set_variant(0)
            _lib.issue_point = prev_hook
        for s in self.streams:
            done = torch.cuda.Event()
            done.record(s)
            caller.wait_event(done)
        if errors:
            raise errors[0]

        def hand_over(obj):
            if isinstance(obj, torch.Tensor):
                if obj.is_cuda:
                    obj.record_stream(caller)
            elif isinstance(obj, (tuple, list)):
                for o in obj:
                    hand_over(o)

        hand_over(results)
        if any(prev_check[:self._n_caller_stacks]):
            self.check_status()
        return results

    def _gemm_variant(self, lib, batches) -> int:
        if not batches:
            return 0
        from myrtlespeech_amd.model.hard_lstm import HardLSTM
        from myrtlespeech_amd.model.rnn import _CELL, RNN
        n = int(batches[0][1].numel())
        wide = []
        for m in self._stacks[:self._n_caller_stacks]:
            if isinstance(m, RNN):
                cell, hidden = _CELL[m.rnn_type], m.rnn.hidden_size
            elif isinstance(m, HardLSTM):
                cell, hidden = _lib.CELL_HARD_LSTM, m.hidden_size
            else:
                return COTENANT_GEMM_VARIANT
            wide.append(bool(lib.ms_rnn_layer_is_wide(int(cell), int(hidden), 2 if m.bidirectional else 1, n)))
        return 0 if wide and all(wide) else COTENANT_GEMM_VARIANT

    def check_status(self):
        lib = _lib.load()
        for m in self._stacks:
            if m._workspace.buf is not None:
                _lib.check(lib.ms_rnn_status(_lib.ptr(m._workspace.buf), _lib.stream_ptr()), "persistent recurrent layer")


class TwoBatchesInFlight(BatchesInFlight):
    def __init__(self, model: torch.nn.Module, post: Optional[Callable] = None, pre: Optional[Callable] = None):
        super().__init__(model, post=post, pre=pre, depth=2)


class PairedBatches:

    def __init__(self, model: torch.nn.Module, post: Optional[Callable] = None, pre: Optional[Callable] = None, max_rows: int = 64):
        _lib.require_gpu()
        self.model, self.post, self.pre, self.max_rows = model, post, pre, max_rows

    def _finish(self, out):
        return out if self.post is None else self.post(out)

    def __call__(self, batches: Sequence) -> List:
        results: List = [None] * len(batches)
        k = 0
        with torch.no_grad():
            while k < len(batches):
                (xa, la) = batches[k]
                pair = None
                if k + 1 < len(batches):
                    (xb, lb) = batches[k + 1]
                    if xa.shape[1:] == xb.shape[1:] and xa.shape[0] + xb.shape[0] <= self.max_rows and xa.dtype == xb.dtype:
                        pair = (xb, lb)
                if pair is None:
                    if self.pre is not None:
                        self.pre(k)
                    results[k] = self._finish(self.model((xa, la)))
                    k += 1
                    continue
                xb, lb = pair
                ha, hb = _lib.host_lens(la), _lib.host_lens(lb)
                na = int(ha.numel())
                both = torch.cat([ha, hb])
                order = torch.sort(both, descending=True, stable=True).indices
                where = torch.empty_like(order)
                where[order] = torch.arange(order.numel())
                dev = xa.device if xa.is_cuda else torch.device("cuda")
                order_d = order.to(dev)
                x = torch.cat([xa.to(dev), xb.to(dev)]).index_select(0, order_d)
                lens = both[order].to(la.dtype)
                if self.pre is not None:
                    self.pre(k)
                    self.pre(k + 1)
                (y, out_lens), hid = self.model((x, lens))
                if bool((both < xa.shape[-1]).any()):
                    back = x.index_select(0, where.to(dev))
                    if xa.is_cuda:
                        xa.copy_(back[:na])
                    if xb.is_cuda:
                        xb.copy_(back[na:])
                out_host = _lib.host_lens(out_lens)
                for b, (lo, hi) in enumerate(((0, na), (na, both.numel()))):
                    pos = where[lo:hi]
                    pos_d = pos.to(dev)
                    lens_b = out_host[pos].to(out_lens.dtype)
                    lens_b = _lib.attach_host(_lib.upload(lens_b), lens_b) if out_lens.is_cuda else lens_b
                    if isinstance(hid, tuple):
                        hid_b = tuple(h.index_select(1, pos_d) for h in hid)
                    else:
                        hid_b = None if hid is None else hid.index_select(1, pos_d)
                    results[k + b] = self._finish(((y.index_select(1, pos_d), lens_b), hid_b))
                k += 2
        return results
```

Before: 27140.

## Add shared-window conv1 kernel writing split planes consumed directly by conv2

Adds a new fwin conv kernel that stages the input window and filters in LDS, shares the window across several output frequency rows, and prefetches filter taps. A paired conv1+conv2 path writes conv1's output straight into channel-last hi/lo fp16 planes, so conv2 skips its own layout and split conversion pass. This removes an intermediate f32 tensor round trip and a transpose kernel. Index uploads in PairedBatches also go through a pinned upload helper. The cost is a new code path with its own LDS budget and tiling limits, and it falls back when a shape is not supported.

After: 28020, median of 6. +3.2%, better.

```diff
diff --git a/include/ms_hotpath.h b/include/ms_hotpath.h
--- a/include/ms_hotpath.h
+++ b/include/ms_hotpath.h
@@ -53,6 +53,19 @@
                              int Fin, int Tin, int Cout, int Fout, int Tout, int KF, int KT, int SF, int ST, int DT,
                              int pad_f_l, int pad_t_l, int act, float act_lo, float act_hi, void* workspace,
                              size_t workspace_bytes, void* stream);
+
+int ms_maskconv_fwin_planes_supported(int N, int Tin, int Cout, int Fout, int Tout, int KF, int KT, int SF, int ST, int DT);
+int ms_maskconv_cl_supported(int N, int Cin, int Fin, int Cout, int Fout, int Tout, int KT, int ST, int DT);
+int ms_maskconv_fwin_planes_forward(const float* x, const int32_t* lens, const void* packed_w, const float* bias, void* planes,
+                                    size_t planes_bytes, int N, int Fin, int Tin, int Cout, int Fout, int Tout, int KF, int KT,
+                                    int SF, int ST, int DT, int pad_f_l, int pad_t_l, int act, float act_lo, float act_hi,
+                                    void* workspace, size_t workspace_bytes, void* stream);
+int ms_maskconv_cl_planes_forward(const int32_t* lens, const void* packed_w, const float* bias, float* y, int N, int Cin,
+                                  int Fin, int Tin, int Cout, int Fout, int Tout, int KF, int KT, int SF, int ST, int DF,
+                                  int DT, int pad_f_l, int pad_t_l, int act, float act_lo, float act_hi, void* planes,
+                                  size_t planes_bytes, void* stream);
+
+int ms_conv_set_variant(int variant);
 
 size_t ms_maskconv1d_gemm_packed_bytes(int Cout, int Cin, int KT);
 int ms_maskconv1d_gemm_pack(const float* w, void* packed, int Cout, int Cin, int KT, void* stream);
diff --git a/myrtlespeech_amd/_lib.py b/myrtlespeech_amd/_lib.py
--- a/myrtlespeech_amd/_lib.py
+++ b/myrtlespeech_amd/_lib.py
@@ -36,6 +36,11 @@
     "ms_maskconv_fwin_pack": (c_int, [_P, _P, c_int, c_int, c_int, _P]),
     "ms_maskconv_fwin_workspace_bytes": (c_size_t, [c_int, c_int, c_int, c_int, c_int]),
     "ms_maskconv_fwin_forward": (c_int, [_P, _P, _P, _P, _P] + [c_int] * 14 + [c_float, c_float, _P, c_size_t, _P]),
+    "ms_maskconv_fwin_planes_forward": (c_int, [_P, _P, _P, _P, _P, c_size_t] + [c_int] * 14 + [c_float, c_float, _P, c_size_t, _P]),
+    "ms_maskconv_cl_planes_forward": (c_int, [_P, _P, _P, _P] + [c_int] * 16 + [c_float, c_float, _P, c_size_t, _P]),
+    "ms_maskconv_fwin_planes_supported": (c_int, [c_int] * 10),
+    "ms_maskconv_cl_supported": (c_int, [c_int] * 9),
+    "ms_conv_set_variant": (c_int, [c_int]),
     "ms_maskconv1d_gemm_packed_bytes": (c_size_t, [c_int, c_int, c_int]),
     "ms_maskconv1d_gemm_pack": (c_int, [_P, _P, c_int, c_int, c_int, _P]),
     "ms_maskconv1d_gemm_workspace_bytes": (c_size_t, [c_int] * 5),
diff --git a/myrtlespeech_amd/csrc/conv_cl.hip b/myrtlespeech_amd/csrc/conv_cl.hip
--- a/myrtlespeech_amd/csrc/conv_cl.hip
+++ b/myrtlespeech_amd/csrc/conv_cl.hip
@@ -20,7 +20,10 @@
   int act;
   float lo, hi;
   int FP;
+  int CS, RG, SG, PQ;
 };
+
+std::atomic<int> g_conv_variant{0};
 
 __device__ __forceinline__ unsigned bf16b(float x) { return (unsigned)__builtin_bit_cast(unsigned short, (__bf16)x); }
 __device__ __forceinline__ unsigned f16b(float x) { return (unsigned)__builtin_bit_cast(unsigned short, (_Float16)x); }
@@ -307,6 +310,216 @@
   return 0;
 }
 
+constexpr int FS_TT = 64;
+constexpr int FS_MR = 5;
+constexpr int FS_TS = 2;
+constexpr int FS_PF = 2;
+
+template <int P>
+__global__ __launch_bounds__(256, 2) void maskconv_fwin_shared_kernel(const unsigned short* __restrict__ xh,
+                                                                      const unsigned short* __restrict__ xl,
+                                                                      const int32_t* __restrict__ lens,
+                                                                      const unsigned short* __restrict__ wp,
+                                                                      const float* __restrict__ bias, float* __restrict__ y,
+                                                                      unsigned short* __restrict__ oh,
+                                                                      unsigned short* __restrict__ ol, ClP p,
+                                                                      const float* __restrict__ scale_word) {
+  constexpr bool F16 = ms::prec_one_plane(P), HM = P == ms::PREC_F16X3;
+  extern __shared__ __attribute__((aligned(16))) char lds[];
+  const int gran_bytes = p.ST * p.PQ * 16;
+  const int in_plane = p.SG * gran_bytes;
+  char* Ph = lds;
+  char* Pl = lds + in_plane;
+  char* Wh = lds + (F16 ? 1 : 2) * in_plane;
+  char* Wl = Wh + FS_TS * p.KG * 32 * 16;
+
+  const int tid = threadIdx.x, lane = tid & 63, wave = tid >> 6;
+  const int l31 = lane & 31, half = lane >> 5;
+  const int fb = wave & 1, rg = wave >> 1;
+  const int t0 = blockIdx.x * FS_TT;
+  const int cls = blockIdx.y % p.CS, jb = blockIdx.y / p.CS;
+  const int fo_first = cls + jb * (2 * FS_MR) * p.CS;
+  if (fo_first >= p.Fout) return;
+  const int nrows = min(2 * FS_MR, (p.Fout - 1 - fo_first) / p.CS + 1);
+  const int n = blockIdx.z / p.co_tiles, tile = blockIdx.z % p.co_tiles;
+  const int len = lens ? min(lens[n], p.Tin) : p.Tin;
+  const int cout_pad = p.co_tiles * 32;
+  const size_t wplane = (size_t)p.KT * p.KG * cout_pad * 8;
+
+  u32x4 fh[FS_PF], fl[FS_PF];
+  auto load_filters = [&](int kt0) {
+    const int ng = min(FS_TS, p.KT - kt0) * p.KG * 32;
+#pragma unroll
+    for (int j = 0; j < FS_PF; ++j) {
+      const int i = tid + 256 * j;
+      if (i < ng) {
+        const int co = i & 31, rest = i >> 5;
+        const size_t src = (((size_t)kt0 * p.KG + rest) * cout_pad + tile * 32 + co) * 8;
+        fh[j] = *reinterpret_cast<const u32x4*>(wp + src);
+        if (!F16) fl[j] = *reinterpret_cast<const u32x4*>(wp + wplane + src);
+      }
+    }
+  };
+  auto store_filters = [&](int kt0) {
+    const int ng = min(FS_TS, p.KT - kt0) * p.KG * 32;
+#pragma unroll
+    for (int j = 0; j < FS_PF; ++j) {
+      const int i = tid + 256 * j;
+      if (i < ng) {
+        *reinterpret_cast<u32x4*>(Wh + i * 16) = fh[j];
+        if (!F16) *reinterpret_cast<u32x4*>(Wl + i * 16) = fl[j];
+      }
+    }
+  };
+  load_filters(0);
+
+  {
+    const unsigned plane_bytes = (unsigned)((size_t)p.N * p.Tin * p.FP * 2);
+    const __amdgpu_buffer_rsrc_t xh_rsrc = __builtin_amdgcn_make_buffer_rsrc(const_cast<unsigned short*>(xh), 0, plane_bytes, 0x00020000);
+    const __amdgpu_buffer_rsrc_t xl_rsrc = __builtin_amdgcn_make_buffer_rsrc(const_cast<unsigned short*>(xl), 0, plane_bytes, 0x00020000);
+    const int tin0 = t0 * p.ST - p.pad_t;
+    const int g = tid & 15;
+    const int span = (nrows - 1) * p.RG + p.KG;
+    if (g < span) {
+      for (int q = tid >> 4; q < p.PW; q += 16) {
+        const int tin = tin0 + q;
+        u32x4 vh = {0u, 0u, 0u, 0u}, vl = {0u, 0u, 0u, 0u};
+        if (tin >= 0 && tin < len) {
+          const int boff = (int)((((size_t)n * p.Tin + tin) * p.FP + (size_t)fo_first * p.SF + g * 8) * 2);
+          vh = __builtin_amdgcn_raw_buffer_load_b128(xh_rsrc, boff, 0, 0);
+          if (!F16) vl = __builtin_amdgcn_raw_buffer_load_b128(xl_rsrc, boff, 0, 0);
+        }
+        const int qq = q / p.ST, qr = q - qq * p.ST;
+        const int off = g * gran_bytes + (qr * p.PQ + qq) * 16;
+        *reinterpret_cast<u32x4*>(Ph + off) = vh;
+        if (!F16) *reinterpret_cast<u32x4*>(Pl + off) = vl;
+      }
+    }
+  }
+  store_filters(0);
+  __syncthreads();
+
+  ms::f32x16 acc[FS_MR];
+#pragma unroll
+  for (int f = 0; f < FS_MR; ++f)
+#pragma unroll
+    for (int r = 0; r < 16; ++r) acc[f][r] = 0.f;
+
+  int row_off[FS_MR];
+#pragma unroll
+  for (int f = 0; f < FS_MR; ++f) row_off[f] = min(rg * FS_MR + f, nrows - 1) * p.RG * gran_bytes;
+
+  for (int kt0 = 0; kt0 < p.KT; kt0 += FS_TS) {
+    const int ntap = min(FS_TS, p.KT - kt0);
+    const bool more = kt0 + FS_TS < p.KT;
+    if (more) load_filters(kt0 + FS_TS);
+    for (int ktl = 0; ktl < ntap; ++ktl) {
+      const int kd = (kt0 + ktl) * p.DT, kq = kd / p.ST, kr = kd - kq * p.ST;
+      const int lane_off = (kr * p.PQ + kq + fb * 32 + l31) * 16;
+      for (int s = 0; s < p.KG / 2; ++s) {
+        const int kg = 2 * s + half;
+        const int woff = ((ktl * p.KG + kg) * 32 + l31) * 16;
+        const u32x4 ah = *reinterpret_cast<const u32x4*>(Wh + woff);
+        u32x4 al = ah;
+        if (!F16) al = *reinterpret_cast<const u32x4*>(Wl + woff);
+#pragma unroll
+        for (int f = 0; f < FS_MR; ++f) {
+          const int poff = row_off[f] + kg * gran_bytes + lane_off;
+          const u32x4 bh = *reinterpret_cast<const u32x4*>(Ph + poff);
+          if (F16) {
+            acc[f] = __builtin_amdgcn_mfma_f32_32x32x16_f16(__builtin_bit_cast(f16x8, ah), __builtin_bit_cast(f16x8, bh), acc[f], 0, 0, 0);
+          } else {
+            const u32x4 bl = *reinterpret_cast<const u32x4*>(Pl + poff);
+            acc[f] = ms::mfma_32x32x16<HM>(ah, bh, acc[f]);
+            acc[f] = ms::mfma_32x32x16<HM>(al, bh, acc[f]);
+            acc[f] = ms::mfma_32x32x16<HM>(ah, bl, acc[f]);
+          }
+        }
+      }
+    }
+    if (more) {
+      __syncthreads();
+      store_filters(kt0 + FS_TS);
+      __syncthreads();
+    }
+  }
+
+  const int t = t0 + fb * 32 + l31;
+  const float winv = scale_word[1];
+  if (t < p.Tout) {
+#pragma unroll
+    for (int f = 0; f < FS_MR; ++f) {
+      const int j = rg * FS_MR + f;
+      if (j >= nrows) continue;
+      const int fo = fo_first + j * p.CS;
+      if (oh) {
+#pragma unroll
+        for (int r4 = 0; r4 < 4; ++r4) {
+          const int co = tile * 32 + ms::mfma32_row(4 * r4, lane);
+          if (co >= p.Cout) continue;
+          unsigned h[4], l[4];
+#pragma unroll
+          for (int e = 0; e < 4; ++e) {
+            float v = acc[f][4 * r4 + e] * winv + (bias ? bias[co + e] : 0.f);
+            if (p.act == MS_ACT_CLAMP) v = fminf(fmaxf(v, p.lo), p.hi);
+            split_by_prec(v, P, h[e], l[e]);
+          }
+          const size_t o = (((size_t)n * p.Fout + fo) * p.Tout + t) * p.Cout + co;
+          *reinterpret_cast<u32x2*>(oh + o) = u32x2{h[0] | (h[1] << 16), h[2] | (h[3] << 16)};
+          if (!F16) *reinterpret_cast<u32x2*>(ol + o) = u32x2{l[0] | (l[1] << 16), l[2] | (l[3] << 16)};
+        }
+        continue;
+      }
+#pragma unroll
+      for (int r = 0; r < 16; ++r) {
+        const int co = tile * 32 + ms::mfma32_row(r, lane);
+        if (co < p.Cout) {
+          float v = acc[f][r] * winv + (bias ? bias[co] : 0.f);
+          if (p.act == MS_ACT_CLAMP) v = fminf(fmaxf(v, p.lo), p.hi);
+          y[(((size_t)n * p.Cout + co) * p.Fout + fo) * p.Tout + t] = v;
+        }
+      }
+    }
+  }
+}
+
+int conv_fs_plan(ClP& p, bool f16, size_t* lds) {
+  if (g_conv_variant.load(std::memory_order_relaxed) != 0 || p.Tout <= 48 || p.SF % 2) return 0;
+  int g = 2 * p.SF, b = 16;
+  while (b) { const int r = g % b; g = b; b = r; }
+  p.CS = 16 / g;
+  p.RG = p.CS * p.SF / 8;
+  p.SG = (2 * FS_MR - 1) * p.RG + p.KG;
+  p.PW = (FS_TT - 1) * p.ST + (p.KT - 1) * p.DT + 1;
+  p.PQ = ms::cdiv(p.PW, p.ST);
+  const int planes = f16 ? 1 : 2;
+  *lds = (size_t)planes * ((size_t)p.SG * p.ST * p.PQ * 16 + (size_t)FS_TS * p.KG * 32 * 16);
+  const long rows_y = (long)p.CS * ms::cdiv(ms::cdiv(p.Fout, p.CS), 2 * FS_MR);
+  if (p.SG > 16 || FS_TS * p.KG * 32 > 256 * FS_PF || *lds > 160 * 1024 || rows_y > 65535 || (long)p.N * p.co_tiles > 65535)
+    return 0;
+  return 1;
+}
+
+int conv_fs_launch(const ClP& p, size_t lds, const unsigned short* xh, const unsigned short* xl, const int32_t* lens,
+                   const void* packed_w, const float* bias, float* y, unsigned short* oh, unsigned short* ol,
+                   hipStream_t stream, const float* scale_word) {
+  static ms::DeviceOnce attr_once;
+  if (attr_once.need()) {
+    MS_HIP(hipFuncSetAttribute((const void*)maskconv_fwin_shared_kernel<ms::PREC_BF16X3>, hipFuncAttributeMaxDynamicSharedMemorySize, 160 * 1024));
+    MS_HIP(hipFuncSetAttribute((const void*)maskconv_fwin_shared_kernel<ms::PREC_F16>, hipFuncAttributeMaxDynamicSharedMemorySize, 160 * 1024));
+    MS_HIP(hipFuncSetAttribute((const void*)maskconv_fwin_shared_kernel<ms::PREC_F16X3>, hipFuncAttributeMaxDynamicSharedMemorySize, 160 * 1024));
+    attr_once.done();
+  }
+  const int prec = ms::split_mode();
+  const dim3 grid(ms::cdiv(p.Tout, FS_TT), p.CS * ms::cdiv(ms::cdiv(p.Fout, p.CS), 2 * FS_MR), p.N * p.co_tiles);
+  const unsigned short* wq = (const unsigned short*)packed_w;
+  auto kern = prec == ms::PREC_F16 ? maskconv_fwin_shared_kernel<ms::PREC_F16>
+              : prec == ms::PREC_F16X3 ? maskconv_fwin_shared_kernel<ms::PREC_F16X3> : maskconv_fwin_shared_kernel<ms::PREC_BF16X3>;
+  hipLaunchKernelGGL(kern, grid, dim3(256), lds, stream, xh, xl, lens, wq, bias, y, oh, ol, p, scale_word);
+  MS_LAUNCH_CHECK();
+  return MS_OK;
+}
+
 __global__ void nchw_to_cl_split_kernel(const float* __restrict__ x, unsigned short* __restrict__ hi,
                                         unsigned short* __restrict__ lo, int C, int F, int T, int prec) {
   __shared__ float tile[32][33];
@@ -445,12 +658,27 @@
   return ms::align_up((size_t)N * Tin * fwin_fp(KF, SF, Fout) * 4, 256);
 }
 
-extern "C" int ms_maskconv_fwin_forward(const float* x, const int32_t* lens, const void* packed_w, const float* bias, float* y,
-                                        int N, int Fin, int Tin, int Cout, int Fout, int Tout, int KF, int KT, int SF, int ST,
-                                        int DT, int pad_f_l, int pad_t_l, int act, float act_lo, float act_hi, void* workspace,
-                                        size_t workspace_bytes, void* stream_) {
+static ClP fwin_params(int N, int Tin, int Cout, int Fout, int Tout, int KF, int KT, int SF, int ST, int DT, int pad_t_l) {
+  ClP p{};
+  p.N = N; p.Cin = fwin_kfp(KF); p.Fin = 1; p.Tin = Tin; p.Cout = Cout; p.Fout = Fout; p.Tout = Tout; p.KF = 1; p.KT = KT;
+  p.SF = SF; p.ST = ST; p.DF = 1; p.DT = DT; p.pad_f = 0; p.pad_t = pad_t_l; p.KG = p.Cin / 8;
+  p.co_tiles = ms::cdiv(Cout, 32);
+  p.FP = fwin_fp(KF, SF, Fout);
+  return p;
+}
+
+static int fwin_route(ClP& p, size_t* lds) {
+  if ((size_t)p.N * p.Tin * p.FP * 2 >= ((size_t)1 << 31)) return 0;
+  if (conv_fs_plan(p, ms::split_mode() == ms::PREC_F16, lds)) return -1;
+  return conv_cl_plan(p, lds);
+}
+
+static int fwin_forward(const float* x, const int32_t* lens, const void* packed_w, const float* bias, float* y, void* planes,
+                        int N, int Fin, int Tin, int Cout, int Fout, int Tout, int KF, int KT, int SF, int ST, int DT,
+                        int pad_f_l, int pad_t_l, int act, float act_lo, float act_hi, void* workspace,
+                        size_t workspace_bytes, void* stream_) {
   ms::ProfScope prof_span(MS_PROF_CONV, (hipStream_t)stream_);
-  MS_REQUIRE(x && packed_w && y && workspace, "null pointer");
+  MS_REQUIRE(x && packed_w && (y || planes) && workspace, "null pointer");
   MS_REQUIRE(N > 0 && Fin > 0 && Tin > 0 && Cout > 0 && Fout > 0 && Tout > 0, "bad shape");
   MS_REQUIRE(KF > 0 && KT > 0 && SF > 0 && ST > 0 && DT > 0 && pad_f_l >= 0 && pad_t_l >= 0, "bad kernel");
   MS_REQUIRE(SF % 2 == 0, "feature stride must be even (4-byte aligned window loads)");
@@ -460,27 +688,66 @@
     return MS_ERR_WORKSPACE;
   }
   hipStream_t stream = (hipStream_t)stream_;
-  ClP p;
-  p.N = N; p.Cin = fwin_kfp(KF); p.Fin = 1; p.Tin = Tin; p.Cout = Cout; p.Fout = Fout; p.Tout = Tout; p.KF = 1; p.KT = KT;
-  p.SF = SF; p.ST = ST; p.DF = 1; p.DT = DT; p.pad_f = 0; p.pad_t = pad_t_l; p.KG = p.Cin / 8;
-  p.co_tiles = ms::cdiv(Cout, 32);
+  ClP p = fwin_params(N, Tin, Cout, Fout, Tout, KF, KT, SF, ST, DT, pad_t_l);
   p.act = act; p.lo = act_lo; p.hi = act_hi;
-  p.FP = fwin_fp(KF, SF, Fout);
   size_t lds = 0;
-  const int wf = conv_cl_plan(p, &lds);
-  if (wf == 0 || (size_t)N * Tin * p.FP * 2 >= ((size_t)1 << 31)) {
-    ms::set_error("ms_maskconv_fwin_forward: shape outside the LDS / grid budget");
+  const int route = fwin_route(p, &lds);
+  if (route == 0 || (planes && route != -1)) {
+    ms::set_error(planes ? "ms_maskconv_fwin_planes_forward: shape not served by the shared-window kernel"
+                         : "ms_maskconv_fwin_forward: shape outside the LDS / grid budget");
     return MS_ERR_UNSUPPORTED;
   }
   unsigned short* xh = (unsigned short*)workspace;
   unsigned short* xl = xh + (size_t)N * Tin * p.FP;
-  const int prec = ms::split_mode();
-  const bool f16 = prec == ms::PREC_F16;
   hipLaunchKernelGGL(ft_to_tf_split_kernel, dim3(ms::cdiv(Tin, 32), ms::cdiv(p.FP, 32), N), dim3(32, 8), 0, stream, x, xh, xl,
-                     Fin, Tin, p.FP, pad_f_l, prec);
+                     Fin, Tin, p.FP, pad_f_l, ms::split_mode());
   MS_LAUNCH_CHECK();
-  return conv_cl_launch<true>(p, wf, lds, xh, xl, lens, packed_w, bias, y, stream,
-                              (const float*)((const char*)packed_w + fwin_plane_bytes(Cout, KF, KT)));
+  const float* scale_word = (const float*)((const char*)packed_w + fwin_plane_bytes(Cout, KF, KT));
+  if (route == -1) {
+    unsigned short* oh = (unsigned short*)planes;
+    unsigned short* ol = oh ? oh + (size_t)N * Cout * Fout * Tout : nullptr;
+    return conv_fs_launch(p, lds, xh, xl, lens, packed_w, bias, y, oh, ol, stream, scale_word);
+  }
+  return conv_cl_launch<true>(p, route, lds, xh, xl, lens, packed_w, bias, y, stream, scale_word);
+}
+
+extern "C" int ms_maskconv_fwin_planes_supported(int N, int Tin, int Cout, int Fout, int Tout, int KF, int KT, int SF, int ST,
+                                                 int DT) {
+  if (N <= 0 || Tin <= 0 || Cout <= 0 || Cout % 16 || Fout <= 0 || Tout <= 0 || KF <= 0 || KT <= 0 || SF <= 0 || SF % 2 ||
+      ST <= 0 || DT <= 0)
+    return 0;
+  ClP p = fwin_params(N, Tin, Cout, Fout, Tout, KF, KT, SF, ST, DT, 0);
+  size_t lds = 0;
+  return fwin_route(p, &lds) == -1;
+}
+
+extern "C" int ms_maskconv_fwin_forward(const float* x, const int32_t* lens, const void* packed_w, const float* bias, float* y,
+                                        int N, int Fin, int Tin, int Cout, int Fout, int Tout, int KF, int KT, int SF, int ST,
+                                        int DT, int pad_f_l, int pad_t_l, int act, float act_lo, float act_hi, void* workspace,
+                                        size_t workspace_bytes, void* stream_) {
+  MS_REQUIRE(y, "null pointer");
+  return fwin_forward(x, lens, packed_w, bias, y, nullptr, N, Fin, Tin, Cout, Fout, Tout, KF, KT, SF, ST, DT, pad_f_l, pad_t_l,
+                      act, act_lo, act_hi, workspace, workspace_bytes, stream_);
+}
+
+extern "C" int ms_maskconv_fwin_planes_forward(const float* x, const int32_t* lens, const void* packed_w, const float* bias,
+                                               void* planes, size_t planes_bytes, int N, int Fin, int Tin, int Cout, int Fout,
+                                               int Tout, int KF, int KT, int SF, int ST, int DT, int pad_f_l, int pad_t_l,
+                                               int act, float act_lo, float act_hi, void* workspace, size_t workspace_bytes,
+                                               void* stream_) {
+  MS_REQUIRE(planes, "null pointer");
+  MS_REQUIRE(Cout > 0 && Cout % 16 == 0, "planes out need Cout % 16 == 0 (the next convolution's k-steps)");
+  if (N <= 0 || Fout <= 0 || Tout <= 0 || planes_bytes < ms_maskconv_cl_workspace_bytes(N, Cout, Fout, Tout)) {
+    ms::set_error("ms_maskconv_fwin_planes_forward: planes buffer too small");
+    return MS_ERR_WORKSPACE;
+  }
+  return fwin_forward(x, lens, packed_w, bias, nullptr, planes, N, Fin, Tin, Cout, Fout, Tout, KF, KT, SF, ST, DT, pad_f_l,
+                      pad_t_l, act, act_lo, act_hi, workspace, workspace_bytes, stream_);
+}
+
+extern "C" int ms_conv_set_variant(int v) {
+  g_conv_variant.store(v, std::memory_order_relaxed);
+  return MS_OK;
 }
 
 static size_t cl_plane_bytes(int Cout, int Cin, int KF, int KT) {
@@ -511,12 +778,22 @@
   return ms::align_up((size_t)N * Cin * Fin * Tin * 4, 256);
 }
 
-extern "C" int ms_maskconv_cl_forward(const float* x, const int32_t* lens, const void* packed_w, const float* bias, float* y,
-                                      int N, int Cin, int Fin, int Tin, int Cout, int Fout, int Tout, int KF, int KT,
-                                      int SF, int ST, int DF, int DT, int pad_f_l, int pad_t_l, int act, float act_lo,
-                                      float act_hi, void* workspace, size_t workspace_bytes, void* stream_) {
+extern "C" int ms_maskconv_cl_supported(int N, int Cin, int Fin, int Cout, int Fout, int Tout, int KT, int ST, int DT) {
+  if (N <= 0 || Cin <= 0 || Cin % 16 || Fin <= 0 || Cout <= 0 || Fout <= 0 || Tout <= 0 || KT <= 0 || ST <= 0 || DT <= 0 ||
+      (long)N * Fin > 65535)
+    return 0;
+  ClP p{};
+  p.N = N; p.Fout = Fout; p.Tout = Tout; p.KT = KT; p.ST = ST; p.DT = DT; p.KG = Cin / 8; p.co_tiles = ms::cdiv(Cout, 32);
+  size_t lds = 0;
+  return conv_cl_plan(p, &lds) != 0;
+}
+
+static int cl_forward(const float* x, const int32_t* lens, const void* packed_w, const float* bias, float* y,
+                      int N, int Cin, int Fin, int Tin, int Cout, int Fout, int Tout, int KF, int KT,
+                      int SF, int ST, int DF, int DT, int pad_f_l, int pad_t_l, int act, float act_lo,
+                      float act_hi, void* workspace, size_t workspace_bytes, void* stream_) {
   ms::ProfScope prof_span(MS_PROF_CONV, (hipStream_t)stream_);
-  MS_REQUIRE(x && packed_w && y && workspace, "null pointer");
+  MS_REQUIRE(packed_w && y && workspace, "null pointer");
   MS_REQUIRE(N > 0 && Cin > 0 && Cin % 16 == 0 && Fin > 0 && Tin > 0 && Cout > 0 && Fout > 0 && Tout > 0, "bad shape");
   MS_REQUIRE(KF > 0 && KT > 0 && SF > 0 && ST > 0 && DF > 0 && DT > 0 && pad_f_l >= 0 && pad_t_l >= 0, "bad kernel");
   MS_REQUIRE(act == MS_ACT_NONE || act == MS_ACT_CLAMP, "bad act");
@@ -531,6 +808,7 @@
   p.co_tiles = ms::cdiv(Cout, 32);
   p.act = act; p.lo = act_lo; p.hi = act_hi;
   p.FP = 0;
+  p.CS = p.RG = p.SG = p.PQ = 0;
   size_t lds = 0;
   const int wf = conv_cl_plan(p, &lds);
   if (wf == 0) {
@@ -543,9 +821,11 @@
   MS_REQUIRE(N * Fin <= 65535, "N*Fin exceeds grid limits");
   const int prec = ms::split_mode();
   const bool f16 = prec == ms::PREC_F16;
-  hipLaunchKernelGGL(nchw_to_cl_split_kernel, dim3(ms::cdiv(Tin, 32), ms::cdiv(Cin, 32), N * Fin), dim3(32, 8), 0, stream, x,
-                     xh, xl, Cin, Fin, Tin, prec);
-  MS_LAUNCH_CHECK();
+  if (x) {
+    hipLaunchKernelGGL(nchw_to_cl_split_kernel, dim3(ms::cdiv(Tin, 32), ms::cdiv(Cin, 32), N * Fin), dim3(32, 8), 0, stream, x,
+                       xh, xl, Cin, Fin, Tin, prec);
+    MS_LAUNCH_CHECK();
+  }
   {
     int RB = 0, RIN = 0;
     size_t slds = 0;
@@ -570,3 +850,20 @@
   }
   return conv_cl_launch<false>(p, wf, lds, xh, xl, lens, packed_w, bias, y, stream, scale_word);
 }
+
+extern "C" int ms_maskconv_cl_forward(const float* x, const int32_t* lens, const void* packed_w, const float* bias, float* y,
+                                      int N, int Cin, int Fin, int Tin, int Cout, int Fout, int Tout, int KF, int KT,
+                                      int SF, int ST, int DF, int DT, int pad_f_l, int pad_t_l, int act, float act_lo,
+                                      float act_hi, void* workspace, size_t workspace_bytes, void* stream_) {
+  MS_REQUIRE(x, "null pointer");
+  return cl_forward(x, lens, packed_w, bias, y, N, Cin, Fin, Tin, Cout, Fout, Tout, KF, KT, SF, ST, DF, DT, pad_f_l, pad_t_l,
+                    act, act_lo, act_hi, workspace, workspace_bytes, stream_);
+}
+
+extern "C" int ms_maskconv_cl_planes_forward(const int32_t* lens, const void* packed_w, const float* bias, float* y, int N,
+                                             int Cin, int Fin, int Tin, int Cout, int Fout, int Tout, int KF, int KT, int SF,
+                                             int ST, int DF, int DT, int pad_f_l, int pad_t_l, int act, float act_lo,
+                                             float act_hi, void* planes, size_t planes_bytes, void* stream_) {
+  return cl_forward(nullptr, lens, packed_w, bias, y, N, Cin, Fin, Tin, Cout, Fout, Tout, KF, KT, SF, ST, DF, DT, pad_f_l,
+                    pad_t_l, act, act_lo, act_hi, planes, planes_bytes, stream_);
+}
diff --git a/myrtlespeech_amd/model/cnn.py b/myrtlespeech_amd/model/cnn.py
--- a/myrtlespeech_amd/model/cnn.py
+++ b/myrtlespeech_amd/model/cnn.py
@@ -93,6 +93,19 @@
         return self.buf
 
 
+def _geometry(x_shape, weight4: torch.Tensor, stride, dilation, same: bool, time_pads: Optional[Tuple[int, int]] = None):
+    _, _, fin, tin = x_shape
+    _, _, kf, kt = weight4.shape
+    (sf, st), (df, dt) = stride, dilation
+    pt = pad_same(tin, kt, st, dt) if same else (0, 0)
+    pf = pad_same(fin, kf, sf, df) if same else (0, 0)
+    if time_pads is not None:
+        pt = (int(time_pads[0]), int(time_pads[1]))
+    fout = (fin + sum(pf) - (df * (kf - 1) + 1)) // sf + 1
+    tout = (tin + sum(pt) - (dt * (kt - 1) + 1)) // st + 1
+    return pf, pt, fout, tout
+
+
 def _conv_forward(x4: torch.Tensor, seq_lens: torch.Tensor, weight4: torch.Tensor, bias: Optional[torch.Tensor],
                   packed: _PackedFilters, stride, dilation, groups: int, same: bool,
                   act: Optional[Tuple[float, float]], time_pads: Optional[Tuple[int, int]] = None):
@@ -100,15 +113,7 @@
     n, cin, fin, tin = x4.shape
     cout, _, kf, kt = weight4.shape
     (sf, st), (df, dt) = stride, dilation
-    if same:
-        pt = pad_same(tin, kt, st, dt)
-        pf = pad_same(fin, kf, sf, df)
-    else:
-        pt = pf = (0, 0)
-    if time_pads is not None:
-        pt = (int(time_pads[0]), int(time_pads[1]))
-    fout = (fin + sum(pf) - (df * (kf - 1) + 1)) // sf + 1
-    tout = (tin + sum(pt) - (dt * (kt - 1) + 1)) // st + 1
+    pf, pt, fout, tout = _geometry(x4.shape, weight4, stride, dilation, same, time_pads)
     if fout <= 0 or tout <= 0:
         raise RuntimeError("convolution output would be empty")
     host_in = _lib.host_lens(seq_lens).to(seq_lens.dtype)
@@ -155,6 +160,71 @@
     return y, new_lens
 
 
+def _has_forward_hooks(m: torch.nn.Module) -> bool:
+    mod = torch.nn.modules.module
+    return bool(m._forward_hooks or m._forward_pre_hooks or mod._global_forward_hooks or mod._global_forward_pre_hooks)
+
+
+def conv_pair_forward(m1: "MaskConv2d", act1: Tuple[float, float], m2: "MaskConv2d", act2: Optional[Tuple[float, float]], x):
+    acts, seq_lens = x
+    if not (_lib.split_precision() and acts.is_cuda and acts.dtype == torch.float32 and acts.dim() == 4):
+        return None
+    if m1.groups != 1 or m2.groups != 1 or os.environ.get("MS_CONV_FWIN") == "0":
+        return None
+    if _has_forward_hooks(m1) or _has_forward_hooks(m2):
+        return None
+    w1, w2 = m1.weight, m2.weight
+    n, cin1, fin1, tin1 = acts.shape
+    cout1, _, kf1, kt1 = w1.shape
+    cout2, cin2, kf2, kt2 = w2.shape
+    (sf1, st1), (df1, dt1) = _pair(m1.stride), _pair(m1.dilation)
+    (sf2, st2), (df2, dt2) = _pair(m2.stride), _pair(m2.dilation)
+    same1, same2 = m1._padding_mode == PaddingMode.SAME, m2._padding_mode == PaddingMode.SAME
+    pf1, pt1, fout1, tout1 = _geometry(acts.shape, w1, (sf1, st1), (df1, dt1), same1)
+    if fout1 <= 0 or tout1 <= 0 or cin1 != 1 or w1.shape[1] != 1 or cin2 != cout1:
+        return None
+    pf2, pt2, fout2, tout2 = _geometry((n, cout1, fout1, tout1), w2, (sf2, st2), (df2, dt2), same2)
+    if fout2 <= 0 or tout2 <= 0:
+        return None
+    flops1 = 2.0 * n * cout1 * fout1 * tout1 * kf1 * kt1
+    flops2 = 2.0 * n * cout2 * fout2 * tout2 * cin2 * kf2 * kt2
+    if not (df1 == 1 and sf1 % 2 == 0 and kf1 >= 16 and flops1 >= float(os.environ.get("MS_CONV_MFMA_MIN_FLOPS", "2e8"))):
+        return None
+    if not (cin2 % 16 == 0 and flops2 >= float(os.environ.get("MS_CONV_MFMA_MIN_FLOPS", "1e9"))):
+        return None
+    if fout1 == 1 and kf2 == 1 and sf2 == 1 and pf2 == (0, 0) and cin2 * kt2 >= 64:
+        return None
+    lib = _lib.load()
+    if not (lib.ms_maskconv_fwin_planes_supported(n, tin1, cout1, fout1, tout1, kf1, kt1, sf1, st1, dt1)
+            and lib.ms_maskconv_cl_supported(n, cin2, fout1, cout2, fout2, tout2, kt2, st2, dt2)):
+        return None
+    _mask_in_place(acts, seq_lens)
+    x4 = _lib.f32c(acts)
+    host0 = _lib.host_lens(seq_lens).to(seq_lens.dtype)
+    host1 = out_lens(host0, kt1, st1, dt1, sum(pt1))
+    host2 = out_lens(host1, kt2, st2, dt2, sum(pt2))
+    pk1, pk2 = m1._packed.get_fwin(w1), m2._packed.get_cl(w2)
+    nbytes1 = lib.ms_maskconv_fwin_workspace_bytes(n, tin1, kf1, sf1, fout1)
+    ws1 = m1._packed.workspace.get(nbytes1)
+    planes = m2._packed.workspace.get(lib.ms_maskconv_cl_workspace_bytes(n, cin2, fout1, tout1))
+    b1 = None if m1.bias is None else _lib.f32c(m1.bias.detach())
+    b2 = None if m2.bias is None else _lib.f32c(m2.bias.detach())
+    lens0_dev = _lib.lens_i32(seq_lens)
+    _lib.check(lib.ms_maskconv_fwin_planes_forward(_lib.ptr(x4), _lib.ptr(lens0_dev), _lib.ptr(pk1), _lib.ptr(b1),
+                                                   _lib.ptr(planes), planes.numel(), n, fin1, tin1, cout1, fout1, tout1, kf1,
+                                                   kt1, sf1, st1, dt1, pf1[0], pt1[0], _lib.ACT_CLAMP, act1[0], act1[1],
+                                                   _lib.ptr(ws1), nbytes1, _lib.stream_ptr()),
+               "ms_maskconv_fwin_planes_forward")
+    lens1_dev = _lib.upload(host1, torch.int32)
+    y = torch.empty((n, cout2, fout2, tout2), dtype=torch.float32, device="cuda")
+    a2, lo2, hi2 = (_lib.ACT_NONE, 0.0, 0.0) if act2 is None else (_lib.ACT_CLAMP, act2[0], act2[1])
+    _lib.check(lib.ms_maskconv_cl_planes_forward(_lib.ptr(lens1_dev), _lib.ptr(pk2), _lib.ptr(b2), _lib.ptr(y), n, cin2, fout1,
+                                                 tout1, cout2, fout2, tout2, kf2, kt2, sf2, st2, df2, dt2, pf2[0], pt2[0], a2,
+                                                 lo2, hi2, _lib.ptr(planes), planes.numel(), _lib.stream_ptr()),
+               "ms_maskconv_cl_planes_forward")
+    return y, _lib.attach_host(_lib.upload(host2), host2)
+
+
 def _mask_in_place(acts: torch.Tensor, seq_lens: torch.Tensor):
     if acts.is_cuda and acts.dtype == torch.float32 and acts.is_contiguous():
         n, t = acts.shape[0], acts.shape[-1]
diff --git a/myrtlespeech_amd/model/deep_speech_2.py b/myrtlespeech_amd/model/deep_speech_2.py
--- a/myrtlespeech_amd/model/deep_speech_2.py
+++ b/myrtlespeech_amd/model/deep_speech_2.py
@@ -3,7 +3,7 @@
 import torch
 
 from myrtlespeech_amd import _lib
-from myrtlespeech_amd.model.cnn import Conv1dTo2d, Conv2dTo1d, MaskConv1d, MaskConv2d
+from myrtlespeech_amd.model.cnn import Conv1dTo2d, Conv2dTo1d, MaskConv1d, MaskConv2d, conv_pair_forward
 from myrtlespeech_amd.model.fully_connected import FullyConnected, linear_stack_plan, run_linear_stack
 from myrtlespeech_amd.model.lookahead import Lookahead, lookahead_apply
 from myrtlespeech_amd.model.rnn import RNNState
@@ -14,6 +14,10 @@
 def _is_plain_activation(m) -> bool:
     return (isinstance(m, SeqLenWrapper) and isinstance(m.module, (torch.nn.Hardtanh, torch.nn.ReLU, torch.nn.Identity))
             and isinstance(m.seq_lens_fn, torch.nn.Identity))
+
+
+def _is_plain_clamp(m) -> bool:
+    return _is_plain_activation(m) and isinstance(m.module, (torch.nn.Hardtanh, torch.nn.ReLU))
 
 
 class DeepSpeech2(torch.nn.Module):
@@ -34,6 +38,15 @@
         i = 0
         while i < len(mods):
             m = mods[i]
+            if (isinstance(m, MaskConv2d) and i + 2 < len(mods) and _is_plain_clamp(mods[i + 1])
+                    and isinstance(mods[i + 2], MaskConv2d)):
+                act2 = i + 3 < len(mods) and _is_plain_activation(mods[i + 3])
+                out = conv_pair_forward(m, activation_clamp(mods[i + 1].module), mods[i + 2],
+                                        activation_clamp(mods[i + 3].module) if act2 else None, h)
+                if out is not None:
+                    h = out
+                    i += 4 if act2 else 3
+                    continue
             if isinstance(m, (MaskConv1d, MaskConv2d)) and i + 1 < len(mods) and _is_plain_activation(mods[i + 1]):
                 h = m(h, fused_activation=activation_clamp(mods[i + 1].module))
                 i += 2
diff --git a/myrtlespeech_amd/pipeline.py b/myrtlespeech_amd/pipeline.py
--- a/myrtlespeech_amd/pipeline.py
+++ b/myrtlespeech_amd/pipeline.py
@@ -163,6 +163,12 @@
 class TwoBatchesInFlight(BatchesInFlight):
     def __init__(self, model: torch.nn.Module, post: Optional[Callable] = None, pre: Optional[Callable] = None):
         super().__init__(model, post=post, pre=pre, depth=2)
+
+
+def _index_to(index: torch.Tensor, dev: torch.device) -> torch.Tensor:
+    if dev.index in (None, torch.cuda.current_device()):
+        return _lib.upload(index)
+    return index.to(dev)
 
 
 class PairedBatches:
@@ -199,7 +205,7 @@
                 where = torch.empty_like(order)
                 where[order] = torch.arange(order.numel())
                 dev = xa.device if xa.is_cuda else torch.device("cuda")
-                order_d = order.to(dev)
+                order_d = _index_to(order, dev)
                 x = torch.cat([xa.to(dev), xb.to(dev)]).index_select(0, order_d)
                 lens = both[order].to(la.dtype)
                 if self.pre is not None:
@@ -207,7 +213,7 @@
                     self.pre(k + 1)
                 (y, out_lens), hid = self.model((x, lens))
                 if bool((both < xa.shape[-1]).any()):
-                    back = x.index_select(0, where.to(dev))
+                    back = x.index_select(0, _index_to(where, dev))
                     if xa.is_cuda:
                         xa.copy_(back[:na])
                     if xb.is_cuda:
@@ -215,7 +221,7 @@
                 out_host = _lib.host_lens(out_lens)
                 for b, (lo, hi) in enumerate(((0, na), (na, both.numel()))):
                     pos = where[lo:hi]
-                    pos_d = pos.to(dev)
+                    pos_d = _index_to(pos, dev)
                     lens_b = out_host[pos].to(out_lens.dtype)
                     lens_b = _lib.attach_host(_lib.upload(lens_b), lens_b) if out_lens.is_cuda else lens_b
                     if isinstance(hid, tuple):
```
